# sevagh/xumx-sliCQ

Measured on AMD Instinct MI355X. Metric: real-time factor (audio-s demixed / wall-s), 44.1 kHz stereo, offline model, higher is better.
Workload: dtype f32; 1 GPU; BASELINE configs[1]: offline model (Bark-262 sliCQT), one 240 s stereo track (10,584,000 samples, 5 chunks) per GPU, Wiener off (mix-phase), seeded synthetic weights; parallelism=one track per rank, 1 rank(s), no data-path collective

## Files before the change

### xumx_slicq_amd/csrc/dft_tables.h

```cpp
#pragma once
namespace xsq {
template <int R> struct DftTw;
template <> struct DftTw<43> {
    static constexpr float c[43] = {1.000000000e+00f, 9.893433681e-01f, 9.576005999e-01f, 9.054482375e-01f, 8.339978179e-01f, 7.447721827e-01f, 6.396730216e-01f, 5.209403405e-01f, 3.911047205e-01f, 2.529333824e-01f, 1.093712084e-01f, -3.652202306e-02f, -1.816368510e-01f, -3.228804048e-01f, -4.572423233e-01f, -5.818589156e-01f, -6.940741952e-01f, -7.914964884e-01f, -8.720494081e-01f, -9.340161087e-01f, -9.760758776e-01f, -9.973322837e-01f, -9.973322837e-01f, -9.760758776e-01f, -9.340161087e-01f, -8.720494081e-01f, -7.914964884e-01f, -6.940741952e-01f, -5.818589156e-01f, -4.572423233e-01f, -3.228804048e-01f, -1.816368510e-01f, -3.652202306e-02f, 1.093712084e-01f, 2.529333824e-01f, 3.911047205e-01f, 5.209403405e-01f, 6.396730216e-01f, 7.447721827e-01f, 8.339978179e-01f, 9.054482375e-01f, 9.576005999e-01f, 9.893433681e-01f};
    static constexpr float s[43] = {0.000000000e+00f, 1.456011677e-01f, 2.880990994e-01f, 4.244566989e-01f, 5.517677408e-01f, 6.673188112e-01f, 7.686471398e-01f, 8.535930890e-01f, 9.203461836e-01f, 9.674836971e-01f, 9.940009752e-01f, 9.993328484e-01f, 9.833656768e-01f, 9.464397732e-01f, 8.893421489e-01f, 8.132897407e-01f, 7.199034738e-01f, 6.111737141e-01f, 4.894178478e-01f, 3.572308898e-01f, 2.174301756e-01f, 7.299531466e-02f, -7.299531466e-02f, -2.174301756e-01f, -3.572308898e-01f, -4.894178478e-01f, -6.111737141e-01f, -7.199034738e-01f, -8.132897407e-01f, -8.893421489e-01f, -9.464397732e-01f, -9.833656768e-01f, -9.993328484e-01f, -9.940009752e-01f, -9.674836971e-01f, -9.203461836e-01f, -8.535930890e-01f, -7.686471398e-01f, -6.673188112e-01f, -5.517677408e-01f, -4.244566989e-01f, -2.880990994e-01f, -1.456011677e-01f};
};
template <> struct DftTw<14> {
    static constexpr float c[14] = {1.000000000e+00f, 9.009688679e-01f, 6.234898019e-01f, 2.225209340e-01f, -2.225209340e-01f, -6.234898019e-01f, -9.009688679e-01f, -1.000000000e+00f, -9.009688679e-01f, -6.234898019e-01f, -2.225209340e-01f, 2.225209340e-01f, 6.234898019e-01f, 9.009688679e-01f};
    static constexpr float s[14] = {0.000000000e+00f, 4.338837391e-01f, 7.818314825e-01f, 9.749279122e-01f, 9.749279122e-01f, 7.818314825e-01f, 4.338837391e-01f, 1.224646799e-16f, -4.338837391e-01f, -7.818314825e-01f, -9.749279122e-01f, -9.749279122e-01f, -7.818314825e-01f, -4.338837391e-01f};
};
template <> struct DftTw<15> {
    static constexpr float c[15] = {1.000000000e+00f, 9.135454576e-01f, 6.691306064e-01f, 3.090169944e-01f, -1.045284633e-01f, -5.000000000e-01f, -8.090169944e-01f, -9.781476007e-01f, -9.781476007e-01f, -8.090169944e-01f, -5.000000000e-01f, -1.045284633e-01f, 3.090169944e-01f, 6.691306064e-01f, 9.135454576e-01f};
    static constexpr float s[15] = {0.000000000e+00f, 4.067366431e-01f, 7.431448255e-01f, 9.510565163e-01f, 9.945218954e-01f, 8.660254038e-01f, 5.877852523e-01f, 2.079116908e-01f, -2.079116908e-01f, -5.877852523e-01f, -8.660254038e-01f, -9.945218954e-01f, -9.510565163e-01f, -7.431448255e-01f, -4.067366431e-01f};
};
template <> struct DftTw<4> {
    static constexpr float c[4] = {1.000000000e+00f, 6.123233996e-17f, -1.000000000e+00f, -1.836970199e-16f};
    static constexpr float s[4] = {0.000000000e+00f, 1.000000000e+00f, 1.224646799e-16f, -1.000000000e+00f};
};
template <> struct DftTw<5> {
    static constexpr float c[5] = {1.000000000e+00f, 3.090169944e-01f, -8.090169944e-01f, -8.090169944e-01f, 3.090169944e-01f};
    static constexpr float s[5] = {0.000000000e+00f, 9.510565163e-01f, 5.877852523e-01f, -5.877852523e-01f, -9.510565163e-01f};
};
template <> struct DftTw<6> {
    static constexpr float c[6] = {1.000000000e+00f, 5.000000000e-01f, -5.000000000e-01f, -1.000000000e+00f, -5.000000000e-01f, 5.000000000e-01f};
    static constexpr float s[6] = {0.000000000e+00f, 8.660254038e-01f, 8.660254038e-01f, 1.224646799e-16f, -8.660254038e-01f, -8.660254038e-01f};
};
template <> struct DftTw<7> {
    static constexpr float c[7] = {1.000000000e+00f, 6.234898019e-01f, -2.225209340e-01f, -9.009688679e-01f, -9.009688679e-01f, -2.225209340e-01f, 6.234898019e-01f};
    static constexpr float s[7] = {0.000000000e+00f, 7.818314825e-01f, 9.749279122e-01f, 4.338837391e-01f, -4.338837391e-01f, -9.749279122e-01f, -7.818314825e-01f};
};
template <> struct DftTw<8> {
    static constexpr float c[8] = {1.000000000e+00f, 7.071067812e-01f, 6.123233996e-17f, -7.071067812e-01f, -1.000000000e+00f, -7.071067812e-01f, -1.836970199e-16f, 7.071067812e-01f};
    static constexpr float s[8] = {0.000000000e+00f, 7.071067812e-01f, 1.000000000e+00f, 7.071067812e-01f, 1.224646799e-16f, -7.071067812e-01f, -1.000000000e+00f, -7.071067812e-01f};
};
template <> struct DftTw<9> {
    static constexpr float c[9] = {1.000000000e+00f, 7.660444431e-01f, 1.736481777e-01f, -5.000000000e-01f, -9.396926208e-01f, -9.396926208e-01f, -5.000000000e-01f, 1.736481777e-01f, 7.660444431e-01f};
    static constexpr float s[9] = {0.000000000e+00f, 6.427876097e-01f, 9.848077530e-01f, 8.660254038e-01f, 3.420201433e-01f, -3.420201433e-01f, -8.660254038e-01f, -9.848077530e-01f, -6.427876097e-01f};
};
template <> struct DftTw<10> {
    static constexpr float c[10] = {1.000000000e+00f, 8.090169944e-01f, 3.090169944e-01f, -3.090169944e-01f, -8.090169944e-01f, -1.000000000e+00f, -8.090169944e-01f, -3.090169944e-01f, 3.090169944e-01f, 8.090169944e-01f};
    static constexpr float s[10] = {0.000000000e+00f, 5.877852523e-01f, 9.510565163e-01f, 9.510565163e-01f, 5.877852523e-01f, 1.224646799e-16f, -5.877852523e-01f, -9.510565163e-01f, -9.510565163e-01f, -5.877852523e-01f};
};
template <> struct DftTw<11> {
    static constexpr float c[11] = {1.000000000e+00f, 8.412535328e-01f, 4.154150130e-01f, -1.423148383e-01f, -6.548607339e-01f, -9.594929736e-01f, -9.594929736e-01f, -6.548607339e-01f, -1.423148383e-01f, 4.154150130e-01f, 8.412535328e-01f};
    static constexpr float s[11] = {0.000000000e+00f, 5.406408175e-01f, 9.096319954e-01f, 9.898214419e-01f, 7.557495744e-01f, 2.817325568e-01f, -2.817325568e-01f, -7.557495744e-01f, -9.898214419e-01f, -9.096319954e-01f, -5.406408175e-01f};
};
template <> struct DftTw<12> {
    static constexpr float c[12] = {1.000000000e+00f, 8.660254038e-01f, 5.000000000e-01f, 6.123233996e-17f, -5.000000000e-01f, -8.660254038e-01f, -1.000000000e+00f, -8.660254038e-01f, -5.000000000e-01f, -1.836970199e-16f, 5.000000000e-01f, 8.660254038e-01f};
    static constexpr float s[12] = {0.000000000e+00f, 5.000000000e-01f, 8.660254038e-01f, 1.000000000e+00f, 8.660254038e-01f, 5.000000000e-01f, 1.224646799e-16f, -5.000000000e-01f, -8.660254038e-01f, -1.000000000e+00f, -8.660254038e-01f, -5.000000000e-01f};
};
template <> struct DftTw<13> {
    static constexpr float c[13] = {1.000000000e+00f, 8.854560257e-01f, 5.680647467e-01f, 1.205366803e-01f, -3.546048870e-01f, -7.485107482e-01f, -9.709418174e-01f, -9.709418174e-01f, -7.485107482e-01f, -3.546048870e-01f, 1.205366803e-01f, 5.680647467e-01f, 8.854560257e-01f};
    static constexpr float s[13] = {0.000000000e+00f, 4.647231720e-01f, 8.229838659e-01f, 9.927088741e-01f, 9.350162427e-01f, 6.631226582e-01f, 2.393156643e-01f, -2.393156643e-01f, -6.631226582e-01f, -9.350162427e-01f, -9.927088741e-01f, -8.229838659e-01f, -4.647231720e-01f};
};
}
```

### xumx_slicq_amd/csrc/plan.h

```cpp
#pragma once
#include <map>
#include <mutex>
#include <tuple>
#include <vector>

#include <rocfft/rocfft.h>

#include "common.h"

namespace xsq {

struct FftPlan {
    rocfft_plan plan = nullptr;
    rocfft_execution_info info = nullptr;
    size_t work_bytes = 0;
};

struct TileTable {
    TileDev* d_tiles = nullptr;
    int ntiles = 0;
};

struct BlockHost {
    int first_band, F, T;
    int64_t cum;
};

}

struct xsq_plan {
    int L = 0, tr = 0, h = 0, nbins = 0, nbands = 0, nblocks = 0;
    int64_t sumFT = 0;
    std::vector<xsq::BandDev> bands;
    std::vector<xsq::BlockHost> blocks;
    int band_radix4 = 1;
    void* d_bands4 = nullptr;
    float* d_pool4f = nullptr;
    float* d_pool4i = nullptr;
    int nbands4 = 0;
    std::vector<unsigned char> bands4_host;
    int64_t d4_max_block = 0;
    std::vector<int> bands4_m, bands4_small;
    int fft_backend = 0;
    float2* d_T = nullptr;
    unsigned short* d_tgt16 = nullptr;
    int* d_tgt = nullptr;
    int phase_begin[5] = {0, 0, 0, 0, 0};
    int packed_fft = 0;
    int short_inline = 0;
    void *d_s_item1 = nullptr, *d_s_tw1 = nullptr;
    int *d_s_item2 = nullptr, *d_s_tgt = nullptr;
    float* d_s_wd = nullptr;
    int short_n1 = 0, short_n2 = 0, short_nent = 0, short_sc0 = 0;
    int short_begin[5] = {0, 0, 0, 0, 0};
    int phase_long[4] = {0, 0, 0, 0};
    float* d_tw = nullptr;
    float* d_Wf = nullptr;
    float* d_Wi = nullptr;
    xsq::BandDev* d_bands = nullptr;
    int* d_cov_ptr = nullptr;
    int* d_cov_band = nullptr;
    std::mutex mu;
    std::map<std::pair<int, int>, xsq::FftPlan> fft;
    std::map<std::tuple<int, int, int>, xsq::TileTable> tiles;
};
```

### xumx_slicq_amd/csrc/slicqt.hip

```cpp
#include <algorithm>
#include <cmath>
#include <cstdarg>
#include <cstdio>
#include <cstdlib>
#include <cstring>

#include "../../include/xumx_slicq_hip.h"
#include "gemm_tile.h"
#include "plan.h"
#include "prof.h"
#include "slice_fft.h"
#include "band_dft4.h"
#include "band_dft4s.h"

namespace xsq {

static thread_local char g_err[1024] = "";
void set_error(const char* fmt, ...) {
    va_list ap;
    va_start(ap, fmt);
    vsnprintf(g_err, sizeof(g_err), fmt, ap);
    va_end(ap);
}

__global__ __launch_bounds__(256) void k_slice_window(const float* __restrict__ x,
                                                       const float* __restrict__ tw,
                                                       float* __restrict__ seg, int S, int64_t n, int L,
                                                       int h, const int64_t* __restrict__ xrows = nullptr,
                                                       const float* const* __restrict__ xslot = nullptr) {
    const int p = blockIdx.x * 256 + threadIdx.x;
    if (p >= L) return;
    const int row = blockIdx.y;
    const int bc = row / S, s = row - bc * S;
    const int64_t i = (int64_t)(2 * s - 2) * h + p;
    float v = 0.f;
    if (i >= 0 && i < n) v = tw[p] * (xslot ? *xslot : x)[(xrows ? xrows[bc] : (int64_t)bc * n) + i];
    seg[(int64_t)row * L + p] = v;
}

__global__ __launch_bounds__(256) void k_spectrum_gather(const float* __restrict__ Z,
                                                          const BandDev* __restrict__ bands,
                                                          const int* __restrict__ cov_ptr,
                                                          const int* __restrict__ cov_band,
                                                          float2* __restrict__ fr, int BC, int S, int nbins) {
    const int k = blockIdx.x * 256 + threadIdx.x;
    if (k >= nbins) return;
    const int row = blockIdx.y;
    const int bc = row / S, s = row - bc * S;
    const int64_t BCS = (int64_t)BC * S;
    float2 acc = make_float2(0.f, 0.f);
    for (int e = cov_ptr[k]; e < cov_ptr[k + 1]; ++e) {
        const BandDev b = bands[cov_band[e]];
        const int64_t off = 2 * (BCS * b.cum + (((int64_t)bc * b.F + b.f) * S + s) * b.Lg + (k - b.bin0));
        const float2 z = *reinterpret_cast<const float2*>(Z + off);
        acc.x += z.x;
        acc.y += z.y;
    }
    if (k == 0 || k == nbins - 1) acc.y = 0.f;
    fr[(int64_t)row * nbins + k] = acc;
}

__global__ __launch_bounds__(256) void k_overlap_add(const float* __restrict__ seg, float* __restrict__ y,
                                                      const int64_t* __restrict__ row_off,
                                                      int S, int64_t length, int L, int h) {
    const int64_t i = (int64_t)blockIdx.x * 256 + threadIdx.x;
    if (i >= length) return;
    const int bc = blockIdx.y;
    const int s0 = (int)(i / (2 * h));
    const int p1 = (int)(i - (int64_t)2 * h * s0);
    const float* base = seg + (int64_t)bc * S * L;
    float v = base[(int64_t)s0 * L + p1 + 2 * h];
    if (s0 + 1 < S) v += base[(int64_t)(s0 + 1) * L + p1];
    y[(row_off ? row_off[bc] : (int64_t)bc * length) + i] = v;
}

struct BandGroup {
    int M, N, K, ldb;
    const float* B;
    int Lg, bin0, f, F;
    int64_t base;
    int64_t cum;
    int j;
};

struct BandFwdOp {
    typedef BandGroup Group;
    struct RowA {
        const float* p;
    };
    const float* U;
    float* coef;
    const BandDev* bands;
    const float* W;
    int BC, S, nbins, L;
    float* xin;
    const float* mean;
    const float* scale;
    int split;

    __device__ Group group(int j) const {
        const BandDev b = bands[j];
        Group g;
        g.M = BC * S; g.N = 2 * b.Lg; g.K = 2 * b.Lg; g.ldb = b.ldw; g.B = W + b.w_off;
        g.Lg = b.Lg; g.bin0 = b.bin0; g.f = b.f; g.F = b.F;
        g.base = 2 * ((int64_t)BC * S * b.cum + (int64_t)b.f * S * b.Lg);
        g.cum = b.cum;
        g.j = j;
        return g;
    }
    __device__ RowA row_a(const Group& g, int m) const {
        RowA r;
        r.p = m < g.M ? U + (int64_t)m * 2 * nbins : nullptr;
        return r;
    }
    __device__ float4 load_a4(const Group& g, const RowA& r, int k) const {
        const bool ok = r.p != nullptr && k < g.K;
        int i0 = g.bin0 + (k >> 1), i1 = i0 + 1;
        i0 = i0 < 0 ? -i0 : (i0 > L / 2 ? L - i0 : i0);
        i1 = i1 < 0 ? -i1 : (i1 > L / 2 ? L - i1 : i1);
        const float2 a = *reinterpret_cast<const float2*>(ok ? r.p + 2 * i0 : zero16());
        const float2 b = *reinterpret_cast<const float2*>(ok ? r.p + 2 * i1 : zero16());
        return make_float4(a.x, a.y, b.x, b.y);
    }
    __device__ void epilogue(const Group& g, int row0, int n, const f32x16& a0, const f32x16& a1, bool wide) const {
        const bool c0 = n < g.N, c1 = wide && n + 32 < g.N;
        int bc = row0 / S, s = row0 - bc * S;
        int prev = 0;
        const float mu = xin ? mean[g.j] : 0.f, sc = xin ? scale[g.j] : 1.f;
#pragma unroll
        for (int r = 0; r < 16; ++r) {
            s += acc_row(r) - prev; prev = acc_row(r);
            while (s >= S) { s -= S; ++bc; }
            if (row0 + acc_row(r) >= g.M) break;
            float* d = coef + g.base + ((int64_t)bc * g.F * S + s) * (2 * g.Lg) + n;
            if (c0) d[0] = a0[r];
            if (c1) d[32] = a1[r];
            if (xin) {
                const float o0 = __shfl_xor(a0[r], 1), o1 = __shfl_xor(a1[r], 1);
                if (!(n & 1)) {
                    float* x = xin + ((d - coef) >> 1);
                    if (c0) { float v = whiten_mag(a0[r], o0, mu, sc); if (split) v = bf3_word(v); x[0] = v; }
                    if (c1) { float v = whiten_mag(a1[r], o1, mu, sc); if (split) v = bf3_word(v); x[16] = v; }
                }
            }
        }
    }
};

struct BandInvOp {
    typedef BandGroup Group;
    struct RowA {
        const float* p;
        const float* mk;
    };
    const float* coef;
    float* Z;
    const BandDev* bands;
    const float* W;
    int BC, S;
    int row_len;
    const float* mask;
    int BCx;

    __device__ Group group(int j) const {
        const BandDev b = bands[j];
        Group g;
        g.M = BC * S; g.N = 2 * b.Lg; g.K = 2 * b.Lg; g.ldb = b.ldw; g.B = W + b.w_off;
        g.Lg = b.Lg; g.bin0 = b.ent; g.f = b.f; g.F = b.F;
        g.base = 2 * ((int64_t)BC * S * b.cum + (int64_t)b.f * S * b.Lg);
        g.cum = b.cum;
        return g;
    }
    __device__ int64_t row_off(const Group& g, int m) const {
        const int bc = m / S, s = m - bc * S;
        return g.base + ((int64_t)bc * g.F * S + s) * (2 * g.Lg);
    }
    __device__ RowA row_a(const Group& g, int m) const {
        RowA r;
        r.p = nullptr; r.mk = nullptr;
        if (m >= g.M) return r;
        if (!mask) { r.p = coef + row_off(g, m); return r; }
        const int bc = m / S, s = m - bc * S;
        r.mk = mask + row_off(g, m) / 2;
        r.p = coef + 2 * ((int64_t)BCx * S * g.cum + (int64_t)g.f * S * g.Lg) + ((int64_t)(bc % BCx) * g.F * S + s) * (2 * g.Lg);
        return r;
    }
    __device__ float4 load_a4(const Group& g, const RowA& r, int k) const {
        const bool ok = r.p != nullptr && k < g.K;
        return *reinterpret_cast<const float4*>(ok ? r.p + k : zero16());
    }
    typedef float2 Aux;
    __device__ Aux load_aux(const Group& g, const RowA& r, int k) const {
        const bool ok = r.mk != nullptr && k < g.K;
        return *reinterpret_cast<const float2*>(ok ? r.mk + (k >> 1) : zero16());
    }
    __device__ float4 finish(float4 v, const Aux& mk) const {
        if (mask) { v.x *= mk.x; v.y *= mk.x; v.z *= mk.y; v.w *= mk.y; }
        return v;
    }
    __device__ void epilogue(const Group& g, int row0, int n, const f32x16& a0, const f32x16& a1, bool wide) const {
        const bool c0 = n < g.N, c1 = wide && n + 32 < g.N;
#pragma unroll
        for (int r = 0; r < 16; ++r) {
            const int m = row0 + acc_row(r);
            if (m >= g.M) break;
            float* d = (row_len ? Z + 2 * ((int64_t)m * row_len + g.bin0) : Z + row_off(g, m)) + n;
            if (c0) d[0] = a0[r];
            if (c1) d[32] = a1[r];
        }
    }
};

constexpr int REMIX_MAX_BLOCKS = 256;
struct RemixArgs {
    const float* src;
    float* dst;
    int nch, R, S, cplx;
    float g[4][4];
    int use[4];
    int cum[REMIX_MAX_BLOCKS + 1];
};

__global__ __launch_bounds__(256) void k_remix_combine(RemixArgs a) {
#pragma clang fp contract(off)
    const int j = blockIdx.y, ch = blockIdx.z;
    const int64_t per = (int64_t)a.S * (a.cum[j + 1] - a.cum[j]) * a.cplx;
    const int64_t e = ((int64_t)blockIdx.x * 256 + threadIdx.x) * 4;
    if (e >= per) return;
    const int64_t base = (int64_t)a.S * a.cum[j] * a.cplx;
    const float* s = a.src + base * (4 * a.nch) + (int64_t)ch * per + e;
    float4 m[4];
#pragma unroll
    for (int t = 0; t < 4; ++t)
        m[t] = a.use[t] ? *reinterpret_cast<const float4*>(s + (int64_t)t * a.nch * per) : make_float4(0.f, 0.f, 0.f, 0.f);
    float* d = a.dst + base * ((int64_t)a.R * a.nch) + (int64_t)ch * per + e;
#pragma unroll
    for (int r = 0; r < 4; ++r) {
        if (r >= a.R) break;
        float4 acc = make_float4(0.f, 0.f, 0.f, 0.f);
#pragma unroll
        for (int t = 0; t < 4; ++t) {
            if (!a.use[t]) continue;
            const float g = a.g[r][t];
            acc.x = acc.x + g * m[t].x; acc.y = acc.y + g * m[t].y; acc.z = acc.z + g * m[t].z; acc.w = acc.w + g * m[t].w;
        }
        *reinterpret_cast<float4*>(d + (int64_t)r * a.nch * per) = acc;
    }
}

static int upload_tiles(const std::vector<TileDev>& t, TileTable* tt) {
    tt->ntiles = (int)t.size();
    tt->d_tiles = nullptr;
    if (t.empty()) return XSQ_OK;
    XSQ_HIP(hipMalloc(&tt->d_tiles, t.size() * sizeof(TileDev)));
    XSQ_HIP(hipMemcpy(tt->d_tiles, t.data(), t.size() * sizeof(TileDev), hipMemcpyHostToDevice));
    return XSQ_OK;
}

static int get_band_tiles(xsq_plan* P, int rows, TileTable* out) {
    std::lock_guard<std::mutex> lk(P->mu);
    const bool r4 = P->band_radix4 && P->nbands4 > 0;
    auto key = std::make_tuple(r4 ? 2 : 0, rows, 0);
    auto it = P->tiles.find(key);
    if (it != P->tiles.end()) { *out = it->second; return XSQ_OK; }
    std::vector<TileDev> t;
    if (r4) {
        for (int i = (int)P->bands4_small.size() - 1; i >= 0; --i)
            push_group_tiles(t, P->bands4_small[i], rows, 2 * P->bands[P->bands4_small[i]].Lg);
    } else {
        for (int j = P->nbands - 1; j >= 0; --j) push_group_tiles(t, j, rows, 2 * P->bands[j].Lg);
    }
    TileTable tt;
    int rc = upload_tiles(t, &tt);
    if (rc) return rc;
    P->tiles[key] = tt;
    *out = tt;
    return XSQ_OK;
}

static int get_dft4_full_tiles(xsq_plan* P, int rows, TileTable* out, int share = 0, int cls = 0, bool sym = false) {
    std::lock_guard<std::mutex> lk(P->mu);
    auto key = std::make_tuple(3 + 16 * cls + (sym ? 256 : 0), rows, share);
    auto it = P->tiles.find(key);
    if (it != P->tiles.end()) { *out = it->second; return XSQ_OK; }
    std::vector<Tile4Dev> t;
    const Band4Dev* b4 = reinterpret_cast<const Band4Dev*>(P->bands4_host.data());
    const int span = share > 0 ? share : rows, copies = share > 0 ? rows / share : 1;
    for (int i = P->nbands4 - 1; i >= 0; --i) {
        int ncb = (2 * P->bands4_m[i] + 15) / 16;
        if ((cls == 1 && ncb <= 5) || (cls == 2 && ncb > 5)) continue;
        if (sym) ncb = (P->bands4_m[i] / 2 + 1 + 15) / 16;
        for (int m0 = 0; m0 < span; m0 += D4H_ROWS)
            for (int k = 0; k < copies; ++k) t.push_back(Tile4Dev{m0 + k * span, ncb, b4[i]});
    }
    TileTable tt;
    tt.ntiles = (int)t.size();
    if (!t.empty()) {
        XSQ_HIP(hipMalloc(&tt.d_tiles, t.size() * sizeof(Tile4Dev)));
        XSQ_HIP(hipMemcpy(tt.d_tiles, t.data(), t.size() * sizeof(Tile4Dev), hipMemcpyHostToDevice));
    }
    P->tiles[key] = tt;
    *out = tt;
    return XSQ_OK;
}

static int d4_ranges_ok(const xsq_plan* P, int64_t rows, const char* who) {
    if (!(P->band_radix4 && P->nbands4)) return XSQ_OK;
    XSQ_REQUIRE(8 * rows * P->d4_max_block < (1ll << 30) && (int64_t)8 * D4H_ROWS * std::max<int64_t>(P->nbins, P->sumFT) < (1ll << 30),
                "%s: %lld rows x %lld coefficients of a band block exceed 2^30 bytes; split the call (fewer stacked chunks)",
                who, (long long)rows, (long long)P->d4_max_block);
    return XSQ_OK;
}

template <bool FWD>
static int launch_dft4(xsq_plan* P, const Band4Args& a4, int rows, int share, hipStream_t stream) {
    static const bool split = getenv("XSQ_D4_SPLIT") && atoi(getenv("XSQ_D4_SPLIT")) == 1;
    static const bool sym = !(getenv("XSQ_D4_SYM") && atoi(getenv("XSQ_D4_SYM")) == 0);
    const bool masked = !FWD && a4.mask != nullptr;
    TileTable t;
    int rc;
    if (sym) {
        if ((rc = get_dft4_full_tiles(P, rows, &t, share, 0, true))) return rc;
        if (!t.ntiles) return XSQ_OK;
        if constexpr (!FWD) {
            if (masked) { hipLaunchKernelGGL((band_dft4s_kernel<false, true>), dim3(t.ntiles), dim3(256), 0, stream, a4, (const Tile4Dev*)t.d_tiles, t.ntiles); return XSQ_OK; }
        }
        hipLaunchKernelGGL((band_dft4s_kernel<FWD, false>), dim3(t.ntiles), dim3(256), 0, stream, a4, (const Tile4Dev*)t.d_tiles, t.ntiles);
        return XSQ_OK;
    }
    auto launch = [&](auto ncbmax) {
        constexpr int N = decltype(ncbmax)::value;
        if (!t.ntiles) return;
        if constexpr (!FWD) {
            if (masked) { hipLaunchKernelGGL((band_dft4_full_kernel<false, N, true>), dim3(t.ntiles), dim3(D4H_NT), 0, stream, a4, (const Tile4Dev*)t.d_tiles, t.ntiles); return; }
        }
        hipLaunchKernelGGL((band_dft4_full_kernel<FWD, N, false>), dim3(t.ntiles), dim3(D4H_NT), 0, stream, a4, (const Tile4Dev*)t.d_tiles, t.ntiles);
    };
    if (!split) {
        if ((rc = get_dft4_full_tiles(P, rows, &t, share, 0))) return rc;
        launch(std::integral_constant<int, 10>{});
        return XSQ_OK;
    }
    if ((rc = get_dft4_full_tiles(P, rows, &t, share, 1))) return rc;
    launch(std::integral_constant<int, 10>{});
    if ((rc = get_dft4_full_tiles(P, rows, &t, share, 2))) return rc;
    launch(std::integral_constant<int, 5>{});
    return XSQ_OK;
}

static int get_fft(xsq_plan* P, int inverse, int batch, FftPlan* out) {
    std::lock_guard<std::mutex> lk(P->mu);
    auto key = std::make_pair(inverse, batch);
    auto it = P->fft.find(key);
    if (it != P->fft.end()) {
        *out = it->second;
        return XSQ_OK;
    }
    static std::once_flag once;
    std::call_once(once, [] { rocfft_setup(); });
    FftPlan f;
    size_t len = (size_t)P->L;
    rocfft_status st = rocfft_plan_create(&f.plan, rocfft_placement_notinplace,
                                          inverse ? rocfft_transform_type_real_inverse
                                                  : rocfft_transform_type_real_forward,
                                          rocfft_precision_single, 1, &len, (size_t)batch, nullptr);
    if (st != rocfft_status_success) {
        set_error("rocfft_plan_create(L=%d, batch=%d, inverse=%d) failed: %d", P->L, batch, inverse, (int)st);
        return XSQ_ERR_FFT;
    }
    rocfft_plan_get_work_buffer_size(f.plan, &f.work_bytes);
    if (rocfft_execution_info_create(&f.info) != rocfft_status_success) {
        set_error("rocfft_execution_info_create failed");
        return XSQ_ERR_FFT;
    }
    P->fft[key] = f;
    *out = f;
    return XSQ_OK;
}

static int run_fft(const FftPlan& f, void* in, void* out, void* work, hipStream_t stream) {
    if (rocfft_execution_info_set_stream(f.info, stream) != rocfft_status_success) {
        set_error("rocfft_execution_info_set_stream failed");
        return XSQ_ERR_FFT;
    }
    if (f.work_bytes) {
        if (rocfft_execution_info_set_work_buffer(f.info, work, f.work_bytes) != rocfft_status_success) {
            set_error("rocfft_execution_info_set_work_buffer failed");
            return XSQ_ERR_FFT;
        }
    }
    void* ib[1] = {in};
    void* ob[1] = {out};
    rocfft_status st = rocfft_execute(f.plan, ib, ob, f.info);
    if (st != rocfft_status_success) {
        set_error("rocfft_execute failed: %d", (int)st);
        return XSQ_ERR_FFT;
    }
    return XSQ_OK;
}

static inline size_t al(size_t x) { return (x + 255) / 256 * 256; }

#ifndef XSQ_D4_MIN_LG_DEFAULT
#define XSQ_D4_MIN_LG_DEFAULT 24
#endif
#ifndef XSQ_FFT_NT_FWD
#define XSQ_FFT_NT_FWD 512
#endif
#ifndef XSQ_FFT_NT_INV
#define XSQ_FFT_NT_INV 512
#endif

static int fft_threads(int inverse) {
    static int u[2] = {-1, -1};
    if (u[0] < 0) {
        int f = XSQ_FFT_NT_FWD, i = XSQ_FFT_NT_INV;
        if (const char* e = getenv("XSQ_FFT_THREADS")) { if (sscanf(e, "%d,%d", &f, &i) < 2) i = f; }
        u[0] = f == 512 ? 512 : 256; u[1] = i == 512 ? 512 : 256;
    }
    return u[inverse ? 1 : 0];
}

static inline bool lds_fft(const xsq_plan* P) { return P->fft_backend == 0 && P->L == FFT_L && P->d_tgt != nullptr; }
static inline FftTables fft_tables(const xsq_plan* P) {
    return FftTables{P->d_T, P->d_T + FFT_R1 * FFT_M1, P->d_T + FFT_R1 * FFT_M1 + FFT_R2 * FFT_R3};
}

}

using namespace xsq;

extern "C" {

int xsq_abi_version(void) { return XSQ_ABI_VERSION; }

#ifndef XSQ_BUILD_ARCH
#define XSQ_BUILD_ARCH "unknown"
#endif
#ifndef XSQ_BUILD_FLAGS
#define XSQ_BUILD_FLAGS ""
#endif
const char* xsq_build_info(void) { return "arch=" XSQ_BUILD_ARCH "; flags=" XSQ_BUILD_FLAGS "; date=" __DATE__ " " __TIME__; }
const char* xsq_last_error(void) { return g_err; }

static int plan_build(xsq_plan* P, int L, int tr, int nbands, const int32_t* Lg, const int32_t* c,
                      const float* g, const double* gd, const float* tw);

int xsq_plan_create(xsq_plan** out, int L, int tr, int nbands, const int32_t* Lg, const int32_t* c,
                    const float* g, const double* gd, const float* tw) {
    XSQ_REQUIRE(out && Lg && c && g && gd && tw, "xsq_plan_create: null argument");
    XSQ_REQUIRE(L > 0 && L % 4 == 0 && tr % 2 == 0 && nbands >= 2, "xsq_plan_create: bad L/tr/nbands");
    xsq_plan* P = new xsq_plan();
    const int rc = plan_build(P, L, tr, nbands, Lg, c, g, gd, tw);
    if (rc != XSQ_OK) {
        xsq_plan_destroy(P);
        return rc;
    }
    *out = P;
    return XSQ_OK;
}

static int plan_build(xsq_plan* P, int L, int tr, int nbands, const int32_t* Lg, const int32_t* c,
                      const float* g, const double* gd, const float* tw) {
    P->L = L; P->tr = tr; P->h = L / 4; P->nbins = L / 2 + 1; P->nbands = nbands;
    int64_t cum = 0;
    for (int j = 0; j < nbands;) {
        int k = j;
        while (k + 1 < nbands && Lg[k + 1] == Lg[j]) ++k;
        P->blocks.push_back(BlockHost{j, k - j + 1, Lg[j], cum});
        cum += (int64_t)(k - j + 1) * Lg[j];
        j = k + 1;
    }
    P->nblocks = (int)P->blocks.size();
    P->sumFT = cum;
    int64_t woff = 0, goff = 0;
    std::vector<int64_t> g_off(nbands);
    for (const BlockHost& b : P->blocks) {
        for (int f = 0; f < b.F; ++f) {
            const int j = b.first_band + f;
            if (Lg[j] % 4 != 0 || c[j] % 2 != 0 || Lg[j] > L / 2) {
                set_error("xsq_plan_create: band %d has Lg=%d c=%d (need Lg%%4==0, c even, Lg<=L/2)", j, Lg[j], c[j]);
                return XSQ_ERR_ARG;
            }
            BandDev d;
            d.Lg = Lg[j]; d.bin0 = c[j] - Lg[j] / 2; d.f = f; d.F = b.F; d.cum = b.cum;
            d.ldw = (int)round_up(2 * Lg[j], 16); d.w_off = woff; d.ent = 0;
            woff += round_up(2 * Lg[j], 64) * d.ldw;
            P->bands.push_back(d);
            g_off[j] = goff;
            goff += Lg[j];
        }
    }
    std::vector<float> Wf((size_t)woff, 0.f), Wi((size_t)woff, 0.f);
    const double PI2 = 6.283185307179586476925286766559;
    for (int j = 0; j < nbands; ++j) {
        const BandDev& d = P->bands[j];
        const int n = d.Lg, ld = d.ldw;
        const double sign = ((c[j] / 2) % 2 == 0) ? 1.0 : -1.0;
        std::vector<double> cs(n), sn(n);
        for (int r = 0; r < n; ++r) { cs[r] = std::cos(PI2 * r / n); sn[r] = std::sin(PI2 * r / n); }
        float* wf = Wf.data() + d.w_off;
        float* wi = Wi.data() + d.w_off;
        for (int p = 0; p < n; ++p) {
            const int q = (p + n / 2) % n;
            const int bin = d.bin0 + p;
            const double conj = (bin < 0 || bin > L / 2) ? -1.0 : 1.0;
            const double ga = (double)g[g_off[j] + q] * sign / n;
            const double gs = gd[g_off[j] + q] * n * sign / L;
            for (int t = 0; t < n; ++t) {
                const int r = (int)(((int64_t)q * t) % n);
                const double wr = ga * cs[r], wim = ga * sn[r];
                wf[(size_t)(2 * t) * ld + 2 * p] = (float)wr;
                wf[(size_t)(2 * t + 1) * ld + 2 * p] = (float)wim;
                wf[(size_t)(2 * t) * ld + 2 * p + 1] = (float)(-conj * wim);
                wf[(size_t)(2 * t + 1) * ld + 2 * p + 1] = (float)(conj * wr);
                const double vr = gs * cs[r], vi = -gs * sn[r];
                wi[(size_t)(2 * p) * ld + 2 * t] = (float)vr;
                wi[(size_t)(2 * p + 1) * ld + 2 * t] = (float)vi;
                wi[(size_t)(2 * p) * ld + 2 * t + 1] = (float)(-vi);
                wi[(size_t)(2 * p + 1) * ld + 2 * t + 1] = (float)vr;
            }
        }
    }
    std::vector<int> cov_ptr(P->nbins + 1, 0), cov_band;
    {
        std::vector<std::vector<int>> cov(P->nbins);
        for (int j = 0; j < nbands; ++j)
            for (int p = 0; p < P->bands[j].Lg; ++p) {
                const int k = P->bands[j].bin0 + p;
                if (k >= 0 && k <= L / 2) cov[k].push_back(j);
            }
        for (int k = 0; k < P->nbins; ++k) {
            cov_ptr[k + 1] = cov_ptr[k] + (int)cov[k].size();
            cov_band.insert(cov_band.end(), cov[k].begin(), cov[k].end());
        }
    }
#define UP(dst, vec, T)                                                                           \
    do {                                                                                          \
        XSQ_HIP(hipMalloc(&(dst), (vec).size() * sizeof(T)));                                     \
        XSQ_HIP(hipMemcpy((dst), (vec).data(), (vec).size() * sizeof(T), hipMemcpyHostToDevice)); \
    } while (0)
    UP(P->d_Wf, Wf, float);
    UP(P->d_Wi, Wi, float);
    UP(P->d_bands, P->bands, BandDev);
    UP(P->d_cov_ptr, cov_ptr, int);
    UP(P->d_cov_band, cov_band, int);
#undef UP
    if (L == FFT_L) {
        auto W = [&](int64_t j) {
            j %= L;
            return make_float2((float)std::cos(PI2 * j / L), (float)(-std::sin(PI2 * j / L)));
        };
        std::vector<float2> T;
        for (int k1 = 0; k1 < FFT_R1; ++k1)
            for (int m = 0; m < FFT_M1; ++m) T.push_back(W(2 * (int64_t)k1 * m));
        for (int k2 = 0; k2 < FFT_R2; ++k2)
            for (int n3 = 0; n3 < FFT_R3; ++n3) T.push_back(W(2 * (int64_t)FFT_R1 * n3 * k2));
        for (int k = 0; k <= FFT_N; ++k) T.push_back(W(k));
        XSQ_HIP(hipMalloc(&P->d_T, T.size() * sizeof(float2)));
        XSQ_HIP(hipMemcpy(P->d_T, T.data(), T.size() * sizeof(float2), hipMemcpyHostToDevice));
        std::vector<int> tgt;
        bool ok = true;
        for (int ph = 0; ph < 4; ++ph) {
            P->phase_begin[ph] = (int)tgt.size();
            int last_end = -(1 << 30);
            for (int j = ph; j < nbands; j += 4) {
                BandDev& b = P->bands[j];
                b.ent = (int)tgt.size();
                const int lo = b.bin0 < 0 ? 0 : b.bin0;
                if (lo < last_end) ok = false;
                last_end = b.bin0 + b.Lg > L / 2 + 1 ? L / 2 + 1 : b.bin0 + b.Lg;
                for (int q = 0; q < b.Lg; ++q) {
                    const int k = b.bin0 + q;
                    tgt.push_back(k >= 0 && k <= L / 2 ? k : -1);
                }
            }
        }
        P->phase_begin[4] = (int)tgt.size();
        if (ok) {
            XSQ_HIP(hipMalloc(&P->d_tgt, tgt.size() * sizeof(int)));
            XSQ_HIP(hipMemcpy(P->d_tgt, tgt.data(), tgt.size() * sizeof(int), hipMemcpyHostToDevice));
            std::vector<unsigned short> t16(tgt.size() + 2, 0xFFFFu);
            for (size_t i = 0; i < tgt.size(); ++i) t16[i] = tgt[i] >= 0 ? (unsigned short)tgt[i] : 0xFFFFu;
            XSQ_HIP(hipMalloc(&P->d_tgt16, t16.size() * sizeof(unsigned short)));
            XSQ_HIP(hipMemcpy(P->d_tgt16, t16.data(), t16.size() * sizeof(unsigned short), hipMemcpyHostToDevice));
            XSQ_HIP(hipMemcpy(P->d_bands, P->bands.data(), P->bands.size() * sizeof(BandDev), hipMemcpyHostToDevice));
        }
    }
    {
        std::vector<Band4Dev> b4;
        std::vector<float> pf, pi;
        int d4_min_lg = XSQ_D4_MIN_LG_DEFAULT;
        if (const char* e = getenv("XSQ_D4_MIN_LG")) d4_min_lg = atoi(e) >= 16 ? atoi(e) : d4_min_lg;
        std::map<int, int64_t> doff, twoff, coff;
        auto alloc2 = [&](size_t n) { size_t o = pf.size(); pf.resize(o + n, 0.f); pi.resize(o + n, 0.f); return (int64_t)o; };
        for (int j = 0; j < nbands; ++j) {
            const BandDev& b = P->bands[j];
            if (b.Lg < d4_min_lg || b.Lg > 4 * D4_MPAD) { P->bands4_small.push_back(j); continue; }
            const int n = b.Lg, m = n / 4;
            Band4Dev d;
            memset(&d, 0, sizeof(d));
            d.Lg = n; d.m = m; d.bin0 = b.bin0; d.f = b.f; d.F = b.F; d.ent = b.ent; d.cum = b.cum; d.jband = j;
            d.ldd = (int)round_up(2 * m, 16);
            if (!doff.count(m)) {
                const int64_t o = alloc2((size_t)round_up(2 * m, 64) * d.ldd);
                doff[m] = o;
                for (int k = 0; k < m; ++k)
                    for (int t1 = 0; t1 < m; ++t1) {
                        const int r = (int)(((int64_t)k * t1) % m);
                        const double cr = std::cos(PI2 * r / m), si = std::sin(PI2 * r / m);
                        for (int dir = 0; dir < 2; ++dir) {
                            std::vector<float>& pool = dir ? pi : pf;
                            const double dre = cr, dim = dir ? -si : si;
                            pool[o + (size_t)(2 * k) * d.ldd + 2 * t1] = (float)dre;
                            pool[o + (size_t)(2 * k) * d.ldd + 2 * t1 + 1] = (float)(-dim);
                            pool[o + (size_t)(2 * k + 1) * d.ldd + 2 * t1] = (float)dim;
                            pool[o + (size_t)(2 * k + 1) * d.ldd + 2 * t1 + 1] = (float)dre;
                        }
                    }
            }
            d.d_off = doff[m];
            d.K2 = m / 2 + 1; d.ldc = (int)round_up(d.K2, 8);
            if (!coff.count(m)) {
                const size_t csz = (size_t)round_up(d.K2, 16) * d.ldc;
                const int64_t o = alloc2(2 * csz);
                coff[m] = o;
                for (int k = 0; k < d.K2; ++k)
                    for (int nn = 0; nn < d.K2; ++nn) {
                        const int r = (int)(((int64_t)k * nn) % m);
                        const double cr = std::cos(PI2 * r / m), si = (nn == 0 || 2 * nn == m) ? 0.0 : std::sin(PI2 * r / m);
                        pf[o + (size_t)k * d.ldc + nn] = (float)cr;
                        pi[o + (size_t)k * d.ldc + nn] = (float)cr;
                        pf[o + csz + (size_t)k * d.ldc + nn] = (float)(-si);
                        pi[o + csz + (size_t)k * d.ldc + nn] = (float)si;
                    }
            }
            d.c_off = coff[m];
            if (!twoff.count(n)) {
                const int mpad = (m + 7) & ~7;
                const int64_t o = alloc2((size_t)3 * mpad * 2);
                twoff[n] = o;
                for (int r = 1; r <= 3; ++r)
                    for (int t1 = 0; t1 < m; ++t1) {
                        const int e = (r * t1) % n;
                        const double cr = std::cos(PI2 * e / n), si = std::sin(PI2 * e / n);
                        pf[o + 2 * ((size_t)(r - 1) * mpad + t1)] = (float)cr;
                        pf[o + 2 * ((size_t)(r - 1) * mpad + t1) + 1] = (float)si;
                        pi[o + 2 * ((size_t)(r - 1) * mpad + t1)] = (float)cr;
                        pi[o + 2 * ((size_t)(r - 1) * mpad + t1) + 1] = (float)(-si);
                    }
            }
            d.tw_off = twoff[n];
            d.win_off = alloc2((size_t)round_up(n, 4));
            const double sign = ((c[j] / 2) % 2 == 0) ? 1.0 : -1.0;
            for (int q = 0; q < n; ++q) {
                pf[d.win_off + q] = (float)((double)g[g_off[j] + q] * sign / n);
                pi[d.win_off + q] = (float)(gd[g_off[j] + q] * n * sign / L);
            }
            b4.push_back(d);
            P->bands4_m.push_back(m);
            P->d4_max_block = std::max<int64_t>(P->d4_max_block, (int64_t)b.F * b.Lg);
        }
        P->nbands4 = (int)b4.size();
        P->bands4_host.assign(reinterpret_cast<const unsigned char*>(b4.data()),
                              reinterpret_cast<const unsigned char*>(b4.data()) + b4.size() * sizeof(Band4Dev));
        if (P->nbands4) {
            XSQ_HIP(hipMalloc(&P->d_bands4, b4.size() * sizeof(Band4Dev)));
            XSQ_HIP(hipMemcpy(P->d_bands4, b4.data(), b4.size() * sizeof(Band4Dev), hipMemcpyHostToDevice));
            XSQ_HIP(hipMalloc(&P->d_pool4f, pf.size() * sizeof(float)));
            XSQ_HIP(hipMemcpy(P->d_pool4f, pf.data(), pf.size() * sizeof(float), hipMemcpyHostToDevice));
            XSQ_HIP(hipMalloc(&P->d_pool4i, pi.size() * sizeof(float)));
            XSQ_HIP(hipMemcpy(P->d_pool4i, pi.data(), pi.size() * sizeof(float), hipMemcpyHostToDevice));
        }
    }
    XSQ_HIP(hipMalloc(&P->d_tw, (size_t)L * sizeof(float)));
    XSQ_HIP(hipMemcpy(P->d_tw, tw, (size_t)L * sizeof(float), hipMemcpyHostToDevice));
    if (P->d_tgt != nullptr && P->nbands4 > 0 && !P->bands4_small.empty()) {
        bool ok = true;
        int nent = 0, maxbin = 0;
        for (int j : P->bands4_small) {
            const BandDev& b = P->bands[j];
            if (b.Lg % 4 != 0 || b.Lg < 16 || b.Lg > 60) ok = false;
            nent += b.Lg;
            maxbin = std::max(maxbin, b.bin0 + b.Lg);
        }
        const int sc0 = 4096;
        if (maxbin >= sc0 || sc0 + nent > FFT_N + 1) ok = false;
        if (ok) {
            std::vector<ShortItem1> item1;
            std::vector<float2> tw1;
            std::vector<std::pair<int, int>> item2;
            std::vector<int> stgt((size_t)nent, -1);
            std::vector<float> swd((size_t)nent, 0.f);
            int sc = 0;
            for (int ph = 0; ph < 4; ++ph) {
                P->short_begin[ph] = sc;
                for (int j : P->bands4_small) {
                    if (j % 4 != ph) continue;
                    const BandDev& b = P->bands[j];
                    const int n = b.Lg, m = n / 4;
                    const double sign = ((c[j] / 2) % 2 == 0) ? 1.0 : -1.0;
                    for (int t1 = 0; t1 < m; ++t1) {
                        item1.push_back(ShortItem1{(int)b.cum, b.F, b.f, n, t1, sc});
                        for (int r = 1; r <= 3; ++r) {
                            const int e = (r * t1) % n;
                            tw1.push_back(make_float2((float)std::cos(PI2 * e / n), (float)(-std::sin(PI2 * e / n))));
                        }
                    }
                    for (int r = 0; r < 4; ++r) {
                        item2.push_back({m, ((sc + r * m) << 4) | m});
                        for (int k = 0; k < m; ++k) {
                            const int q = 4 * k + r;
                            const int bin = b.bin0 + (q + n / 2) % n;
                            stgt[sc + r * m + k] = (bin >= 0 && bin <= L / 2) ? bin : -1;
                            swd[sc + r * m + k] = (float)(gd[g_off[j] + q] * n * sign / L);
                        }
                    }
                    sc += n;
                }
            }
            P->short_begin[4] = sc;
            std::stable_sort(item2.begin(), item2.end(), [](const std::pair<int, int>& a, const std::pair<int, int>& b) { return a.first < b.first; });
            std::vector<int> codes;
            for (auto& it : item2) codes.push_back(it.second);
            for (int ph = 0; ph < 4; ++ph) {
                int lo = P->phase_begin[ph + 1];
                for (int j = ph; j < nbands; j += 4) {
                    bool is_short = false;
                    for (int js : P->bands4_small) is_short = is_short || js == j;
                    if (!is_short) { lo = P->bands[j].ent; break; }
                }
                P->phase_long[ph] = lo;
                for (int j = ph; j < nbands; j += 4) {
                    bool is_short = false;
                    for (int js : P->bands4_small) is_short = is_short || js == j;
                    if (is_short && P->bands[j].ent >= lo) ok = false;
                }
            }
            if (ok && item1.size() <= 1280 && codes.size() <= 768 && sc <= nent) {
                bool fits = true;
                for (int ph = 0; ph < 4; ++ph) fits = fits && (P->short_begin[ph + 1] - P->short_begin[ph] <= 1280);
                if (fits) {
#define UPV(dst, vec, T)                                                                          \
    do {                                                                                          \
        XSQ_HIP(hipMalloc((void**)&(dst), (vec).size() * sizeof(T)));                             \
        XSQ_HIP(hipMemcpy((dst), (vec).data(), (vec).size() * sizeof(T), hipMemcpyHostToDevice)); \
    } while (0)
                    UPV(P->d_s_item1, item1, ShortItem1);
                    UPV(P->d_s_tw1, tw1, float2);
                    UPV(P->d_s_item2, codes, int);
                    UPV(P->d_s_tgt, stgt, int);
                    UPV(P->d_s_wd, swd, float);
#undef UPV
                    P->short_n1 = (int)item1.size(); P->short_n2 = (int)codes.size();
                    P->short_nent = nent; P->short_sc0 = sc0;
                }
            }
        }
    }
    return XSQ_OK;
}

int xsq_plan_destroy(xsq_plan* P) {
    if (!P) return XSQ_OK;
    for (auto& kv : P->fft) {
        if (kv.second.info) rocfft_execution_info_destroy(kv.second.info);
        if (kv.second.plan) rocfft_plan_destroy(kv.second.plan);
    }
    for (auto& kv : P->tiles) (void)hipFree(kv.second.d_tiles);
    (void)hipFree(P->d_bands4); (void)hipFree(P->d_pool4f); (void)hipFree(P->d_pool4i);
    (void)hipFree(P->d_T); (void)hipFree(P->d_tgt); (void)hipFree(P->d_tgt16); (void)hipFree(P->d_tw); (void)hipFree(P->d_Wf); (void)hipFree(P->d_Wi); (void)hipFree(P->d_bands);
    (void)hipFree(P->d_cov_ptr); (void)hipFree(P->d_cov_band);
    (void)hipFree(P->d_s_item1); (void)hipFree(P->d_s_tw1); (void)hipFree(P->d_s_item2); (void)hipFree(P->d_s_tgt); (void)hipFree(P->d_s_wd);
    delete P;
    return XSQ_OK;
}

int xsq_plan_num_blocks(const xsq_plan* P) { return P ? P->nblocks : XSQ_ERR_ARG; }

int xsq_plan_set_band_radix4(xsq_plan* P, int on) {
    XSQ_REQUIRE(P, "xsq_plan_set_band_radix4: null plan");
    P->band_radix4 = on ? 1 : 0;
    return XSQ_OK;
}

#if XSQ_D4_STAMP
extern "C" int xsq_debug_d4_stamps(unsigned long long* host, int tiles) {
    XSQ_HIP(hipDeviceSynchronize());
    XSQ_HIP(hipMemcpyFromSymbol(host, HIP_SYMBOL(g_d4_stamps), (size_t)(tiles < D4_STAMP_TILES ? tiles : D4_STAMP_TILES) * 64));
    return XSQ_OK;
}
#endif
#if XSQ_FFT_STAMP
extern "C" int xsq_debug_fft_stamps(unsigned long long* host, int rows) {
    XSQ_HIP(hipDeviceSynchronize());
    XSQ_HIP(hipMemcpyFromSymbol(host, HIP_SYMBOL(g_fft_stamps), (size_t)(rows < FFT_STAMP_ROWS ? rows : FFT_STAMP_ROWS) * 64));
    return XSQ_OK;
}
#endif

int xsq_plan_set_packed_fft(xsq_plan* P, int on) {
    XSQ_REQUIRE(P, "xsq_plan_set_packed_fft: null plan");
#if !XSQ_PACKED_FFT_KERNELS
    XSQ_REQUIRE(!on, "xsq_plan_set_packed_fft: this library is built without the packed-fp32 slice FFT kernels "
                "(diagnostic build: make PACKED_FFT=1)");
#endif
    P->packed_fft = on ? 1 : 0;
    return XSQ_OK;
}

int xsq_plan_set_short_inline(xsq_plan* P, int on) {
    XSQ_REQUIRE(P, "xsq_plan_set_short_inline: null plan");
    P->short_inline = on ? 1 : 0;
    return XSQ_OK;
}

int xsq_plan_set_fft_backend(xsq_plan* P, int backend) {
    XSQ_REQUIRE(P && (backend == 0 || backend == 1), "xsq_plan_set_fft_backend: backend must be 0 (auto) or 1 (rocFFT)");
    P->fft_backend = backend;
    return XSQ_OK;
}

int xsq_plan_block_table(const xsq_plan* P, int64_t* table) {
    XSQ_REQUIRE(P && table, "xsq_plan_block_table: null argument");
    for (int b = 0; b < P->nblocks; ++b) {
        table[4 * b + 0] = P->blocks[b].first_band;
        table[4 * b + 1] = P->blocks[b].F;
        table[4 * b + 2] = P->blocks[b].T;
        table[4 * b + 3] = P->blocks[b].cum;
    }
    return XSQ_OK;
}

int64_t xsq_plan_coefs_per_slice(const xsq_plan* P) { return P ? P->sumFT : XSQ_ERR_ARG; }

int xsq_plan_num_slices(const xsq_plan* P, int64_t n) {
    if (!P || n <= 0) return XSQ_ERR_ARG;
    const int64_t nb = (n + P->h - 1) / P->h;
    return (int)((nb + 1) / 2 + 1);
}

size_t xsq_slicqt_forward_workspace(xsq_plan* P, int BC, int64_t n) {
    if (!P || BC <= 0 || n <= 0) return 0;
    const size_t rows = (size_t)BC * xsq_plan_num_slices(P, n);
    FftPlan f;
    if (!lds_fft(P) && get_fft(P, 0, (int)rows, &f)) return 0;
    return al(rows * P->L * 4) + al(rows * P->nbins * 8) + al(f.work_bytes) + 256;
}

int xsq_slicqt_forward(xsq_plan* P, const float* x, int BC, int64_t n, float* coef, void* ws,
                       size_t ws_bytes, void* stream_) {
    return xsq_slicqt_forward_xin(P, x, BC, n, coef, nullptr, nullptr, nullptr, 0, ws, ws_bytes, stream_);
}

int xsq_slicqt_forward_xin(xsq_plan* P, const float* x, int BC, int64_t n, float* coef, float* xin, const float* mean,
                           const float* scale, int split, void* ws, size_t ws_bytes, void* stream_) {
    return xsq_slicqt_forward_rows(P, x, nullptr, BC, n, n, coef, xin, mean, scale, split, ws, ws_bytes, stream_);
}

int xsq_slicqt_forward_rows(xsq_plan* P, const float* x, const int64_t* x_rows, int BC, int64_t n, int64_t n_pad, float* coef,
                            float* xin, const float* mean, const float* scale, int split, void* ws, size_t ws_bytes,
                            void* stream_) {
    XSQ_REQUIRE(x, "xsq_slicqt_forward: null argument");
    return xsq_slicqt_forward_rows_indirect(P, x, nullptr, x_rows, BC, n, n_pad, coef, xin, mean, scale, split, ws, ws_bytes, stream_);
}

int xsq_slicqt_forward_rows_indirect(xsq_plan* P, const float* x, const float* const* x_slot, const int64_t* x_rows, int BC, int64_t n,
                                     int64_t n_pad, float* coef, float* xin, const float* mean, const float* scale, int split,
                                     void* ws, size_t ws_bytes, void* stream_) {
    XSQ_REQUIRE(P && (x || x_slot) && coef && ws, "xsq_slicqt_forward: null argument");
    XSQ_REQUIRE(!xin || (mean && scale), "xsq_slicqt_forward_xin: xin needs the mean / scale tables");
    XSQ_REQUIRE(BC > 0 && n > 0 && n_pad >= n, "xsq_slicqt_forward: BC=%d n=%lld n_pad=%lld", BC, (long long)n, (long long)n_pad);
    hipStream_t stream = (hipStream_t)stream_;
    const int S = xsq_plan_num_slices(P, n_pad);
    const int rows = BC * S;
    XSQ_REQUIRE(S >= 2, "xsq_slicqt_forward: signal too short");
    XSQ_REQUIRE((int64_t)BC * S <= 65535, "xsq_slicqt_forward: BC*S=%lld rows exceed one launch", (long long)BC * S);
    XSQ_REQUIRE((int64_t)2 * BC * S * (P->sumFT > P->nbins ? P->sumFT : P->nbins) < (1ll << 31),
                "xsq_slicqt_forward: BC*S=%lld rows exceed 2^31 floats of coefficients; split the call", (long long)BC * S);
    if (int rcg = d4_ranges_ok(P, (int64_t)BC * S, "xsq_slicqt_forward")) return rcg;
    FftPlan f;
    int rc = lds_fft(P) ? XSQ_OK : get_fft(P, 0, rows, &f);
    if (rc) return rc;
    char* w = (char*)ws;
    float* seg = (float*)w; w += al((size_t)rows * P->L * 4);
    float* U = (float*)w;   w += al((size_t)rows * P->nbins * 8);
    void* fwork = w;
    if ((size_t)(w - (char*)ws) + f.work_bytes > ws_bytes) {
        set_error("xsq_slicqt_forward: workspace too small (%zu needed, %zu given)",
                  (size_t)(w - (char*)ws) + f.work_bytes, ws_bytes);
        return XSQ_ERR_WORKSPACE;
    }
    if (lds_fft(P)) {
        XSQ_PROF("slice_rfft", stream);
#if XSQ_PACKED_FFT_KERNELS
        if (fft_threads(0) == 512 && P->packed_fft) hipLaunchKernelGGL((k_slice_rfft<512, true>), dim3(rows), dim3(512), 0, stream, x, P->d_tw, fft_tables(P), (float2*)U, S, n, P->h, x_rows, x_slot);
        else
#endif
        if (fft_threads(0) == 512) hipLaunchKernelGGL(k_slice_rfft<512>, dim3(rows), dim3(512), 0, stream, x, P->d_tw, fft_tables(P), (float2*)U, S, n, P->h, x_rows, x_slot);
        else hipLaunchKernelGGL(k_slice_rfft<256>, dim3(rows), dim3(256), 0, stream, x, P->d_tw, fft_tables(P), (float2*)U, S, n, P->h, x_rows, x_slot);
    } else {
        { XSQ_PROF("slice_window", stream);
        hipLaunchKernelGGL(k_slice_window, dim3((P->L + 255) / 256, rows), dim3(256), 0, stream, x, P->d_tw, seg,
                           S, n, P->L, P->h, x_rows, x_slot); }
        { XSQ_PROF("rfft_L", stream); rc = run_fft(f, seg, U, fwork, stream); }
        if (rc) return rc;
    }
    TileTable tt;
    rc = get_band_tiles(P, rows, &tt);
    if (rc) return rc;
    BandFwdOp op{U, coef, P->d_bands, P->d_Wf, BC, S, P->nbins, P->L, xin, mean, scale, split};
    if (P->band_radix4 && P->nbands4) {
        Band4Args a4{(const Band4Dev*)P->d_bands4, P->d_pool4f, U, coef, BC, S, P->nbins, P->L, 0, nullptr, 0, xin, mean, scale, split};
        XSQ_PROF("band_analysis_dft4", stream);
        if ((rc = launch_dft4<true>(P, a4, rows, 0, stream))) return rc;
    }
    if (tt.ntiles) { XSQ_PROF("band_analysis_gemm", stream);
    hipLaunchKernelGGL((grouped_gemm_kernel<BandFwdOp>), dim3(tt.ntiles), dim3(256), 0, stream, op,
                       tt.d_tiles, tt.ntiles); }
    XSQ_HIP(hipGetLastError());
    return XSQ_OK;
}

size_t xsq_slicqt_inverse_workspace(xsq_plan* P, int BC, int S) {
    if (!P || BC <= 0 || S <= 0) return 0;
    const size_t rows = (size_t)BC * S;
    FftPlan f;
    if (!lds_fft(P) && get_fft(P, 1, (int)rows, &f)) return 0;
    if (lds_fft(P)) return al(rows * P->sumFT * 8) + 256;
    return al(rows * P->sumFT * 8) + al(rows * P->nbins * 8) + al(rows * P->L * 4) + al(f.work_bytes) + 256;
}

int xsq_slicqt_inverse(xsq_plan* P, const float* coef, int BC, int S, int64_t length, float* y, void* ws,
                       size_t ws_bytes, void* stream_) {
    return xsq_slicqt_inverse_rows(P, coef, BC, S, length, y, nullptr, ws, ws_bytes, stream_);
}

static int inverse_impl(xsq_plan* P, const float* coef, const float* mask, int BCx, int BC, int S, int64_t length, float* y,
                        const int64_t* row_offsets, void* ws, size_t ws_bytes, void* stream_);

int xsq_slicqt_inverse_rows(xsq_plan* P, const float* coef, int BC, int S, int64_t length, float* y,
                            const int64_t* row_offsets, void* ws, size_t ws_bytes, void* stream_) {
    return inverse_impl(P, coef, nullptr, 0, BC, S, length, y, row_offsets, ws, ws_bytes, stream_);
}

int xsq_slicqt_inverse_masked(xsq_plan* P, const float* masks, const float* mix, int BC, int BCx, int S, int64_t length,
                              float* y, const int64_t* row_offsets, void* ws, size_t ws_bytes, void* stream_) {
    XSQ_REQUIRE(masks && mix, "xsq_slicqt_inverse_masked: null argument");
    XSQ_REQUIRE(BCx > 0 && BC % BCx == 0, "xsq_slicqt_inverse_masked: %d mix channels do not divide %d mask channels", BCx, BC);
    return inverse_impl(P, mix, masks, BCx, BC, S, length, y, row_offsets, ws, ws_bytes, stream_);
}

static int inverse_impl(xsq_plan* P, const float* coef, const float* mask, int BCx, int BC, int S, int64_t length, float* y,
                        const int64_t* row_offsets, void* ws, size_t ws_bytes, void* stream_) {
    XSQ_REQUIRE(P && coef && y && ws, "xsq_slicqt_inverse: null argument");
    XSQ_REQUIRE(BC > 0 && S >= 2 && length > 0, "xsq_slicqt_inverse: BC=%d S=%d length=%lld", BC, S,
                (long long)length);
    XSQ_REQUIRE(length <= (int64_t)2 * S * P->h, "xsq_slicqt_inverse: length %lld exceeds the %d slices",
                (long long)length, S);
    XSQ_REQUIRE((int64_t)BC * S <= 65535, "xsq_slicqt_inverse: BC*S=%lld rows exceed one launch", (long long)BC * S);
    XSQ_REQUIRE((int64_t)2 * BC * S * P->sumFT < (1ll << 31), "xsq_slicqt_inverse: the coefficient arena of BC*S=%lld rows "
                "exceeds 2^31 floats; split the call (fewer stacked chunks)", (long long)BC * S);
    if (int rcg = d4_ranges_ok(P, (int64_t)BC * S, "xsq_slicqt_inverse")) return rcg;
    hipStream_t stream = (hipStream_t)stream_;
    const int rows = BC * S;
    FftPlan f;
    int rc = lds_fft(P) ? XSQ_OK : get_fft(P, 1, rows, &f);
    if (rc) return rc;
    char* w = (char*)ws;
    float* Z = (float*)w;    w += al((size_t)rows * P->sumFT * 8);
    float2* fr = (float2*)w; if (!lds_fft(P)) w += al((size_t)rows * P->nbins * 8);
    float* seg = (float*)w;  if (!lds_fft(P)) w += al((size_t)rows * P->L * 4);
    void* fwork = w;
    if ((size_t)(w - (char*)ws) + f.work_bytes > ws_bytes) {
        set_error("xsq_slicqt_inverse: workspace too small (%zu needed, %zu given)",
                  (size_t)(w - (char*)ws) + f.work_bytes, ws_bytes);
        return XSQ_ERR_WORKSPACE;
    }
    TileTable tt;
    rc = get_band_tiles(P, rows, &tt);
    if (rc) return rc;
    BandInvOp op{coef, Z, P->d_bands, P->d_Wi, BC, S, lds_fft(P) ? (int)P->sumFT : 0, mask, BCx};
    if (P->band_radix4 && P->nbands4) {
        Band4Args a4{(const Band4Dev*)P->d_bands4, P->d_pool4i, coef, Z, BC, S, P->nbins, P->L,
                     lds_fft(P) ? (int)P->sumFT : 0, mask, BCx, nullptr, nullptr, nullptr, 0};
        XSQ_PROF("band_synthesis_dft4", stream);
        if ((rc = launch_dft4<false>(P, a4, rows, mask ? BCx * S : 0, stream))) return rc;
    }
    const bool inl = lds_fft(P) && P->band_radix4 && P->short_inline && P->short_n1 > 0;
    if (tt.ntiles && !inl) { XSQ_PROF("band_synthesis_gemm", stream);
    hipLaunchKernelGGL((grouped_gemm_kernel<BandInvOp>), dim3(tt.ntiles), dim3(256), 0, stream, op,
                       tt.d_tiles, tt.ntiles); }
    if (lds_fft(P)) {
        XSQ_PROF("slice_irfft_ola", stream);
        GatherSched G;
        G.tgt = P->d_tgt; G.tgt16 = P->d_tgt16; G.row_len = (int)P->sumFT;
        for (int i = 0; i < 5; ++i) G.begin[i] = P->phase_begin[i];
        for (int i = 0; i < 4; ++i) G.lo[i] = inl ? P->phase_long[i] : P->phase_begin[i];
        ShortSched SS;
        memset(&SS, 0, sizeof(SS));
        if (inl) {
            SS.item1 = (const ShortItem1*)P->d_s_item1; SS.tw1 = (const float2*)P->d_s_tw1; SS.item2 = P->d_s_item2;
            SS.stgt = P->d_s_tgt; SS.swd = P->d_s_wd;
            SS.n1 = P->short_n1; SS.n2 = P->short_n2; SS.nent = P->short_nent; SS.sc0 = P->short_sc0;
            for (int i = 0; i < 5; ++i) SS.begin[i] = P->short_begin[i];
        }
        const ShortIn SI{coef, mask, BC, mask ? BCx : BC};
        for (int parity = 0; parity < 2; ++parity) {
            const int nsl = (S + 1 - parity) / 2;
            OlaArgs O{y, row_offsets, S, P->h, parity, length};
            const bool sh = SS.n1 > 0;
            bool fast4 = !sh && fft_threads(1) == 512 && G.tgt16 != nullptr && !getenv("XSQ_FFT_GATHER2");
            for (int ph = 0; ph < 4; ++ph) fast4 = fast4 && (G.begin[ph + 1] - (G.lo[ph] & ~1) <= 2 * 512 * ((4864 / 2 + 1 + 511) / 512));
#if XSQ_PACKED_FFT_KERNELS
            if (fast4 && P->packed_fft) hipLaunchKernelGGL((k_slice_irfft<512, true, false, true>), dim3(BC * nsl), dim3(512), 0, stream, (const float2*)Z, G, fft_tables(P), O, SS, SI);
            else if (!fast4 && !sh && fft_threads(1) == 512 && P->packed_fft) hipLaunchKernelGGL((k_slice_irfft<512, true>), dim3(BC * nsl), dim3(512), 0, stream, (const float2*)Z, G, fft_tables(P), O, SS, SI);
            else
#endif
            if (fast4) hipLaunchKernelGGL((k_slice_irfft<512, false, false, true>), dim3(BC * nsl), dim3(512), 0, stream, (const float2*)Z, G, fft_tables(P), O, SS, SI);
            else if (fft_threads(1) == 512 && sh) hipLaunchKernelGGL((k_slice_irfft<512, false, true>), dim3(BC * nsl), dim3(512), 0, stream, (const float2*)Z, G, fft_tables(P), O, SS, SI);
            else if (fft_threads(1) == 512) hipLaunchKernelGGL(k_slice_irfft<512>, dim3(BC * nsl), dim3(512), 0, stream, (const float2*)Z, G, fft_tables(P), O, SS, SI);
            else if (sh) hipLaunchKernelGGL((k_slice_irfft<256, false, true>), dim3(BC * nsl), dim3(256), 0, stream, (const float2*)Z, G, fft_tables(P), O, SS, SI);
            else hipLaunchKernelGGL(k_slice_irfft<256>, dim3(BC * nsl), dim3(256), 0, stream, (const float2*)Z, G, fft_tables(P), O, SS, SI);
        }
        XSQ_HIP(hipGetLastError());
        return XSQ_OK;
    } else {
        { XSQ_PROF("spectrum_gather", stream);
        hipLaunchKernelGGL(k_spectrum_gather, dim3((P->nbins + 255) / 256, rows), dim3(256), 0, stream, Z,
                           P->d_bands, P->d_cov_ptr, P->d_cov_band, fr, BC, S, P->nbins); }
        { XSQ_PROF("irfft_L", stream); rc = run_fft(f, fr, seg, fwork, stream); }
        if (rc) return rc;
    }
    { XSQ_PROF("overlap_add", stream);
    hipLaunchKernelGGL(k_overlap_add, dim3((unsigned)((length + 255) / 256), BC), dim3(256), 0, stream, seg, y,
                       row_offsets, S, length, P->L, P->h); }
    XSQ_HIP(hipGetLastError());
    return XSQ_OK;
}

static int remix_gains_ok(const float* gains, int R, const char* who) {
    XSQ_REQUIRE(gains, "%s: null gains", who);
    XSQ_REQUIRE(R >= 1 && R <= 4, "%s: R=%d mixes (1..4)", who, R);
    for (int i = 0; i < 4 * R; ++i) XSQ_REQUIRE(std::isfinite(gains[i]), "%s: gain [%d][%d] is not finite", who, i / 4, i % 4);
    return XSQ_OK;
}

size_t xsq_slicqt_remix_workspace(xsq_plan* P, int R, int B, int S, int wiener) {
    if (!P || R < 1 || R > 4 || B <= 0 || S <= 0) return 0;
    const size_t inv = xsq_slicqt_inverse_workspace(P, R * 2 * B, S);
    if (!inv) return 0;
    return al((size_t)R * 2 * B * S * P->sumFT * (wiener ? 8 : 4)) + inv;
}

int xsq_slicqt_inverse_remix(xsq_plan* P, const float* masks, const float* mix, const float* Y, const float* gains, int R, int B,
                             int S, int64_t length, float* y, const int64_t* row_offsets, void* ws, size_t ws_bytes, void* stream_) {
    if (int rc = remix_gains_ok(gains, R, "xsq_slicqt_inverse_remix")) return rc;
    XSQ_REQUIRE(P && y && ws, "xsq_slicqt_inverse_remix: null argument");
    XSQ_REQUIRE(Y ? (!masks && !mix) : (masks && mix), "xsq_slicqt_inverse_remix: pass masks and mix (mix-phase) or Y (Wiener-EM), not both");
    XSQ_REQUIRE(B > 0 && S >= 2 && 2 * B <= 65535, "xsq_slicqt_inverse_remix: B=%d S=%d", B, S);
    XSQ_REQUIRE(P->nblocks <= REMIX_MAX_BLOCKS, "xsq_slicqt_inverse_remix: %d band blocks (at most %d)", P->nblocks, REMIX_MAX_BLOCKS);
    const int wiener = Y ? 1 : 0, BC = R * 2 * B;
    const size_t need = xsq_slicqt_remix_workspace(P, R, B, S, wiener);
    XSQ_REQUIRE(need && need <= ws_bytes, "xsq_slicqt_inverse_remix: workspace too small (%zu needed, %zu given)", need, ws_bytes);
    const size_t comb_bytes = al((size_t)BC * S * P->sumFT * (wiener ? 8 : 4));
    float* comb = (float*)ws;
    RemixArgs a;
    a.src = Y ? Y : masks; a.dst = comb; a.nch = 2 * B; a.R = R; a.S = S; a.cplx = wiener ? 2 : 1;
    for (int t = 0; t < 4; ++t) a.use[t] = 0;
    for (int r = 0; r < 4; ++r)
        for (int t = 0; t < 4; ++t) {
            a.g[r][t] = r < R ? gains[4 * r + t] : 0.f;
            if (r < R && gains[4 * r + t] != 0.f) a.use[t] = 1;
        }
    int64_t per_max = 0;
    for (int j = 0; j < P->nblocks; ++j) {
        a.cum[j] = (int)P->blocks[j].cum;
        per_max = std::max<int64_t>(per_max, (int64_t)S * P->blocks[j].F * P->blocks[j].T * a.cplx);
    }
    a.cum[P->nblocks] = (int)P->sumFT;
    hipStream_t stream = (hipStream_t)stream_;
    { XSQ_PROF("remix_combine", stream);
    hipLaunchKernelGGL(k_remix_combine, dim3((unsigned)((per_max / 4 + 255) / 256), P->nblocks, 2 * B), dim3(256), 0, stream, a); }
    XSQ_HIP(hipGetLastError());
    char* inv_ws = (char*)ws + comb_bytes;
    if (wiener) return inverse_impl(P, comb, nullptr, 0, BC, S, length, y, row_offsets, inv_ws, ws_bytes - comb_bytes, stream_);
    return inverse_impl(P, mix, comb, 2 * B, BC, S, length, y, row_offsets, inv_ws, ws_bytes - comb_bytes, stream_);
}

}
```

Measured before the change: 55340 x real-time.

## Add register/LDS radix-4 FFT kernel for mid-size bands in inverse synthesis

Adds a wave-per-16-rows kernel that computes the inverse band transform for bands of length 16 to 60 as a radix-4 by small-DFT factorisation, using per-wave LDS staging and compile-time twiddles. Those bands are taken out of the dense GEMM and dft4 tile tables on the synthesis path, replacing an O(n^2) matrix product with an FFT. The change adds a new kernel launch, per-m template instantiations with extra register pressure, and new tile tables keyed on the mask-sharing layout.

```diff
diff --git a/xumx_slicq_amd/csrc/band_fft_reg.h b/xumx_slicq_amd/csrc/band_fft_reg.h
--- /dev/null
+++ b/xumx_slicq_amd/csrc/band_fft_reg.h
@@ -0,0 +1,142 @@
+#pragma once
+#include "band_dft4.h"
+#include "slice_fft.h"
+
+#ifndef XSQ_BAND_REGFFT_MAX_LG
+#define XSQ_BAND_REGFFT_MAX_LG 60
+#endif
+#ifndef XSQ_BAND_REGFFT_ABL
+#define XSQ_BAND_REGFFT_ABL 0
+#endif
+
+namespace xsq {
+
+constexpr int RF_WROWS = 16, RF_WAVES = 4, RF_ROWS = RF_WROWS * RF_WAVES;
+constexpr int RF_MAX_LG = 60, RF_LDS_W = RF_WROWS * (RF_MAX_LG + 1);
+static_assert(XSQ_BAND_REGFFT_MAX_LG <= RF_MAX_LG, "dft_small codelets exist for m <= 15");
+
+__device__ __forceinline__ void rf_wave_sync() {
+    __builtin_amdgcn_fence(__ATOMIC_RELEASE, "wavefront");
+    __builtin_amdgcn_wave_barrier();
+    __builtin_amdgcn_fence(__ATOMIC_ACQUIRE, "wavefront");
+}
+
+template <bool MASKED, int M_>
+__device__ __forceinline__ void band_fft_reg_body(const Band4Args& a, const Tile4Dev& t, float2* __restrict__ lw, int lane, int w0, int nrows) {
+#pragma clang fp contract(off)
+    constexpr int Lg = 4 * M_, LD = Lg + 1, HP = Lg / 2;
+    constexpr int NP = (RF_WROWS * HP + 63) / 64;
+    constexpr bool FULL = NP * 64 == RF_WROWS * HP;
+    const Band4Dev& bd = t.bd;
+    const int M = a.BC * a.S;
+    const int64_t BCS = (int64_t)a.BC * a.S;
+    const unsigned blk = (unsigned)(bd.F * Lg) * (unsigned)a.S;
+
+    const int myrow = t.m0 + w0 + (lane & 15);
+    const bool my_ok = (lane & 15) < nrows && myrow < M;
+    const int rowc = my_ok ? myrow : 0;
+    const int bc = rowc / a.S, sl = rowc - bc * a.S;
+    const unsigned o_arena = my_ok ? 8u * (unsigned)(((bc * bd.F + bd.f) * a.S + sl) * Lg) : BUF_OOB;
+    unsigned o_src = o_arena, o_msk = BUF_OOB;
+    if (MASKED) {
+        o_src = my_ok ? 8u * (unsigned)((((bc % a.BCx) * bd.F + bd.f) * a.S + sl) * Lg) : BUF_OOB;
+        o_msk = my_ok ? 4u * (unsigned)(((bc * bd.F + bd.f) * a.S + sl) * Lg) : BUF_OOB;
+    }
+    const bool rowmajor = a.row_len != 0;
+    const unsigned o_dst = rowmajor ? (my_ok ? 8u * (unsigned)((w0 + (lane & 15)) * a.row_len) : BUF_OOB) : o_arena;
+    const float* const win = a.pool + bd.win_off;
+
+    const __amdgpu_buffer_rsrc_t rx = MASKED ? buf_rsrc(a.src + 2 * ((int64_t)a.BCx * a.S * bd.cum), 8u * a.BCx * blk)
+                                             : buf_rsrc(a.src + 2 * (BCS * bd.cum), 8u * a.BC * blk);
+    const __amdgpu_buffer_rsrc_t rm = MASKED ? buf_rsrc(a.mask + BCS * bd.cum, 4u * a.BC * blk) : buf_rsrc(a.src, 0);
+    float4 v[NP];
+    float2 mk[NP];
+    float2 wd[NP];
+#pragma unroll
+    for (int u = 0; u < NP; ++u) {
+        const int i = lane + 64 * u, row = i / HP, pr = i - row * HP;
+        const bool ok = FULL || i < RF_WROWS * HP;
+        const unsigned ro = (unsigned)__shfl((int)o_src, row & 15);
+        v[u] = buf_ld4(rx, ok ? ro + 16u * (unsigned)pr : BUF_OOB, 0);
+        wd[u] = *reinterpret_cast<const float2*>(win + 2 * pr);
+        if (MASKED) {
+            const unsigned mo = (unsigned)__shfl((int)o_msk, row & 15);
+            mk[u] = buf_ld2(rm, ok ? mo + 8u * (unsigned)pr : BUF_OOB, 0);
+        }
+    }
+#pragma unroll
+    for (int u = 0; u < NP; ++u) {
+        const int i = lane + 64 * u, row = i / HP, pr = i - row * HP;
+        if (!FULL && i >= RF_WROWS * HP) continue;
+        float4 x = v[u];
+        if (MASKED) { x.x *= mk[u].x; x.y *= mk[u].x; x.z *= mk[u].y; x.w *= mk[u].y; }
+        lw[row * LD + 2 * pr] = make_float2(x.x, x.y);
+        lw[row * LD + 2 * pr + 1] = make_float2(x.z, x.w);
+    }
+    rf_wave_sync();
+
+    const int lrow = lane >> 2, r = lane & 3;
+    const bool odd = r & 1;
+    const float s2 = odd ? -1.f : 1.f;
+    const float cx = odd ? (r == 3 ? -1.f : 1.f) : (r == 2 ? -1.f : 1.f);
+    const float cy = odd ? (r == 3 ? 1.f : -1.f) : (r == 2 ? -1.f : 1.f);
+    const float f0 = r == 0 ? 1.f : 0.f, f1 = r == 1 ? 1.f : 0.f, f2 = r == 2 ? 1.f : 0.f, f3 = r == 3 ? 1.f : 0.f;
+    float2* const xr = lw + lrow * LD;
+    float2 y[M_];
+    static_for<0, M_>([&](auto t1c) {
+        constexpr int t1 = t1c;
+        const float2 x0 = xr[t1], x1 = xr[M_ + t1], x2 = xr[2 * M_ + t1], x3 = xr[3 * M_ + t1];
+        const float2 uu = make_float2(fmaf(s2, x2.x, x0.x), fmaf(s2, x2.y, x0.y));
+        const float2 vv = make_float2(fmaf(s2, x3.x, x1.x), fmaf(s2, x3.y, x1.y));
+        const float pp = odd ? vv.y : vv.x, qq = odd ? vv.x : vv.y;
+        const float2 yy = make_float2(fmaf(cx, pp, uu.x), fmaf(cy, qq, uu.y));
+        if constexpr (t1 == 0) {
+            y[t1] = yy;
+        } else {
+            constexpr float c1 = DftTw<Lg>::c[t1], c2 = DftTw<Lg>::c[2 * t1 % Lg], c3 = DftTw<Lg>::c[3 * t1 % Lg];
+            constexpr float s1 = -DftTw<Lg>::s[t1], s2_ = -DftTw<Lg>::s[2 * t1 % Lg], s3 = -DftTw<Lg>::s[3 * t1 % Lg];
+            const float wx = fmaf(f1, c1, fmaf(f2, c2, fmaf(f3, c3, f0)));
+            const float wy = fmaf(f1, s1, fmaf(f2, s2_, f3 * s3));
+            y[t1] = make_float2(fmaf(yy.x, wx, -(yy.y * wy)), fmaf(yy.x, wy, yy.y * wx));
+        }
+    });
+    rf_wave_sync();
+    dft_small<M_, -1>(y, [&](int k, float2 X) {
+        const int q = 4 * k + r;
+        xr[q < 2 * M_ ? q + 2 * M_ : q - 2 * M_] = X;
+    });
+    rf_wave_sync();
+
+    const float* const dbase = rowmajor ? a.dst + 2 * ((int64_t)t.m0 * a.row_len + bd.ent) : a.dst + 2 * (BCS * bd.cum);
+    const unsigned dbytes = rowmajor ? 8u * (unsigned)(RF_ROWS * a.row_len) : 8u * a.BC * blk;
+    const __amdgpu_buffer_rsrc_t rd = buf_rsrc(dbase, dbytes);
+#pragma unroll
+    for (int u = 0; u < NP; ++u) {
+        const int i = lane + 64 * u, row = i / HP, pr = i - row * HP;
+        const unsigned ro = (unsigned)__shfl((int)o_dst, row & 15);
+        if (!FULL && i >= RF_WROWS * HP) continue;
+        const float2 c0 = lw[row * LD + 2 * pr], c1 = lw[row * LD + 2 * pr + 1];
+        const float4 o = make_float4(c0.x * wd[u].x, c0.y * wd[u].x, c1.x * wd[u].y, c1.y * wd[u].y);
+        buf_st4(o, rd, ro + 16u * (unsigned)pr, 0);
+    }
+}
+
+template <bool MASKED>
+__global__ __launch_bounds__(64 * RF_WAVES) __attribute__((amdgpu_waves_per_eu(4)))
+void band_fft_reg_kernel(Band4Args a, const Tile4Dev* __restrict__ tiles, int ntiles) {
+    __shared__ __attribute__((aligned(16))) float2 lds[RF_WAVES * RF_LDS_W];
+    const int lane = threadIdx.x & 63, wave = threadIdx.x >> 6;
+    const Tile4Dev t = tiles[xcd_remap(blockIdx.x, ntiles)];
+    const int w0 = RF_WROWS * wave, nrows = t.ncb - w0;
+    if (nrows <= 0) return;
+    float2* const lw = lds + wave * RF_LDS_W;
+    switch (t.bd.m) {
+#define XSQ_RF_CASE(MM) case MM: band_fft_reg_body<MASKED, MM>(a, t, lw, lane, w0, nrows); break;
+        XSQ_RF_CASE(4) XSQ_RF_CASE(5) XSQ_RF_CASE(6) XSQ_RF_CASE(7) XSQ_RF_CASE(8) XSQ_RF_CASE(9)
+        XSQ_RF_CASE(10) XSQ_RF_CASE(11) XSQ_RF_CASE(12) XSQ_RF_CASE(13) XSQ_RF_CASE(14) XSQ_RF_CASE(15)
+#undef XSQ_RF_CASE
+        default: break;
+    }
+}
+
+}
diff --git a/xumx_slicq_amd/csrc/dft_tables.h b/xumx_slicq_amd/csrc/dft_tables.h
--- a/xumx_slicq_amd/csrc/dft_tables.h
+++ b/xumx_slicq_amd/csrc/dft_tables.h
@@ -53,4 +53,52 @@
     static constexpr float c[13] = {1.000000000e+00f, 8.854560257e-01f, 5.680647467e-01f, 1.205366803e-01f, -3.546048870e-01f, -7.485107482e-01f, -9.709418174e-01f, -9.709418174e-01f, -7.485107482e-01f, -3.546048870e-01f, 1.205366803e-01f, 5.680647467e-01f, 8.854560257e-01f};
     static constexpr float s[13] = {0.000000000e+00f, 4.647231720e-01f, 8.229838659e-01f, 9.927088741e-01f, 9.350162427e-01f, 6.631226582e-01f, 2.393156643e-01f, -2.393156643e-01f, -6.631226582e-01f, -9.350162427e-01f, -9.927088741e-01f, -8.229838659e-01f, -4.647231720e-01f};
 };
+template <> struct DftTw<16> {
+    static constexpr float c[16] = {1.000000000e+00f, 9.238795325e-01f, 7.071067812e-01f, 3.826834324e-01f, 6.123233996e-17f, -3.826834324e-01f, -7.071067812e-01f, -9.238795325e-01f, -1.000000000e+00f, -9.238795325e-01f, -7.071067812e-01f, -3.826834324e-01f, -1.836970199e-16f, 3.826834324e-01f, 7.071067812e-01f, 9.238795325e-01f};
+    static constexpr float s[16] = {0.000000000e+00f, 3.826834324e-01f, 7.071067812e-01f, 9.238795325e-01f, 1.000000000e+00f, 9.238795325e-01f, 7.071067812e-01f, 3.826834324e-01f, 1.224646799e-16f, -3.826834324e-01f, -7.071067812e-01f, -9.238795325e-01f, -1.000000000e+00f, -9.238795325e-01f, -7.071067812e-01f, -3.826834324e-01f};
+};
+template <> struct DftTw<20> {
+    static constexpr float c[20] = {1.000000000e+00f, 9.510565163e-01f, 8.090169944e-01f, 5.877852523e-01f, 3.090169944e-01f, 6.123233996e-17f, -3.090169944e-01f, -5.877852523e-01f, -8.090169944e-01f, -9.510565163e-01f, -1.000000000e+00f, -9.510565163e-01f, -8.090169944e-01f, -5.877852523e-01f, -3.090169944e-01f, -1.836970199e-16f, 3.090169944e-01f, 5.877852523e-01f, 8.090169944e-01f, 9.510565163e-01f};
+    static constexpr float s[20] = {0.000000000e+00f, 3.090169944e-01f, 5.877852523e-01f, 8.090169944e-01f, 9.510565163e-01f, 1.000000000e+00f, 9.510565163e-01f, 8.090169944e-01f, 5.877852523e-01f, 3.090169944e-01f, 1.224646799e-16f, -3.090169944e-01f, -5.877852523e-01f, -8.090169944e-01f, -9.510565163e-01f, -1.000000000e+00f, -9.510565163e-01f, -8.090169944e-01f, -5.877852523e-01f, -3.090169944e-01f};
+};
+template <> struct DftTw<24> {
+    static constexpr float c[24] = {1.000000000e+00f, 9.659258263e-01f, 8.660254038e-01f, 7.071067812e-01f, 5.000000000e-01f, 2.588190451e-01f, 6.123233996e-17f, -2.588190451e-01f, -5.000000000e-01f, -7.071067812e-01f, -8.660254038e-01f, -9.659258263e-01f, -1.000000000e+00f, -9.659258263e-01f, -8.660254038e-01f, -7.071067812e-01f, -5.000000000e-01f, -2.588190451e-01f, -1.836970199e-16f, 2.588190451e-01f, 5.000000000e-01f, 7.071067812e-01f, 8.660254038e-01f, 9.659258263e-01f};
+    static constexpr float s[24] = {0.000000000e+00f, 2.588190451e-01f, 5.000000000e-01f, 7.071067812e-01f, 8.660254038e-01f, 9.659258263e-01f, 1.000000000e+00f, 9.659258263e-01f, 8.660254038e-01f, 7.071067812e-01f, 5.000000000e-01f, 2.588190451e-01f, 1.224646799e-16f, -2.588190451e-01f, -5.000000000e-01f, -7.071067812e-01f, -8.660254038e-01f, -9.659258263e-01f, -1.000000000e+00f, -9.659258263e-01f, -8.660254038e-01f, -7.071067812e-01f, -5.000000000e-01f, -2.588190451e-01f};
+};
+template <> struct DftTw<28> {
+    static constexpr float c[28] = {1.000000000e+00f, 9.749279122e-01f, 9.009688679e-01f, 7.818314825e-01f, 6.234898019e-01f, 4.338837391e-01f, 2.225209340e-01f, 6.123233996e-17f, -2.225209340e-01f, -4.338837391e-01f, -6.234898019e-01f, -7.818314825e-01f, -9.009688679e-01f, -9.749279122e-01f, -1.000000000e+00f, -9.749279122e-01f, -9.009688679e-01f, -7.818314825e-01f, -6.234898019e-01f, -4.338837391e-01f, -2.225209340e-01f, -1.836970199e-16f, 2.225209340e-01f, 4.338837391e-01f, 6.234898019e-01f, 7.818314825e-01f, 9.009688679e-01f, 9.749279122e-01f};
+    static constexpr float s[28] = {0.000000000e+00f, 2.225209340e-01f, 4.338837391e-01f, 6.234898019e-01f, 7.818314825e-01f, 9.009688679e-01f, 9.749279122e-01f, 1.000000000e+00f, 9.749279122e-01f, 9.009688679e-01f, 7.818314825e-01f, 6.234898019e-01f, 4.338837391e-01f, 2.225209340e-01f, 1.224646799e-16f, -2.225209340e-01f, -4.338837391e-01f, -6.234898019e-01f, -7.818314825e-01f, -9.009688679e-01f, -9.749279122e-01f, -1.000000000e+00f, -9.749279122e-01f, -9.009688679e-01f, -7.818314825e-01f, -6.234898019e-01f, -4.338837391e-01f, -2.225209340e-01f};
+};
+template <> struct DftTw<32> {
+    static constexpr float c[32] = {1.000000000e+00f, 9.807852804e-01f, 9.238795325e-01f, 8.314696123e-01f, 7.071067812e-01f, 5.555702330e-01f, 3.826834324e-01f, 1.950903220e-01f, 6.123233996e-17f, -1.950903220e-01f, -3.826834324e-01f, -5.555702330e-01f, -7.071067812e-01f, -8.314696123e-01f, -9.238795325e-01f, -9.807852804e-01f, -1.000000000e+00f, -9.807852804e-01f, -9.238795325e-01f, -8.314696123e-01f, -7.071067812e-01f, -5.555702330e-01f, -3.826834324e-01f, -1.950903220e-01f, -1.836970199e-16f, 1.950903220e-01f, 3.826834324e-01f, 5.555702330e-01f, 7.071067812e-01f, 8.314696123e-01f, 9.238795325e-01f, 9.807852804e-01f};
+    static constexpr float s[32] = {0.000000000e+00f, 1.950903220e-01f, 3.826834324e-01f, 5.555702330e-01f, 7.071067812e-01f, 8.314696123e-01f, 9.238795325e-01f, 9.807852804e-01f, 1.000000000e+00f, 9.807852804e-01f, 9.238795325e-01f, 8.314696123e-01f, 7.071067812e-01f, 5.555702330e-01f, 3.826834324e-01f, 1.950903220e-01f, 1.224646799e-16f, -1.950903220e-01f, -3.826834324e-01f, -5.555702330e-01f, -7.071067812e-01f, -8.314696123e-01f, -9.238795325e-01f, -9.807852804e-01f, -1.000000000e+00f, -9.807852804e-01f, -9.238795325e-01f, -8.314696123e-01f, -7.071067812e-01f, -5.555702330e-01f, -3.826834324e-01f, -1.950903220e-01f};
+};
+template <> struct DftTw<36> {
+    static constexpr float c[36] = {1.000000000e+00f, 9.848077530e-01f, 9.396926208e-01f, 8.660254038e-01f, 7.660444431e-01f, 6.427876097e-01f, 5.000000000e-01f, 3.420201433e-01f, 1.736481777e-01f, 6.123233996e-17f, -1.736481777e-01f, -3.420201433e-01f, -5.000000000e-01f, -6.427876097e-01f, -7.660444431e-01f, -8.660254038e-01f, -9.396926208e-01f, -9.848077530e-01f, -1.000000000e+00f, -9.848077530e-01f, -9.396926208e-01f, -8.660254038e-01f, -7.660444431e-01f, -6.427876097e-01f, -5.000000000e-01f, -3.420201433e-01f, -1.736481777e-01f, -1.836970199e-16f, 1.736481777e-01f, 3.420201433e-01f, 5.000000000e-01f, 6.427876097e-01f, 7.660444431e-01f, 8.660254038e-01f, 9.396926208e-01f, 9.848077530e-01f};
+    static constexpr float s[36] = {0.000000000e+00f, 1.736481777e-01f, 3.420201433e-01f, 5.000000000e-01f, 6.427876097e-01f, 7.660444431e-01f, 8.660254038e-01f, 9.396926208e-01f, 9.848077530e-01f, 1.000000000e+00f, 9.848077530e-01f, 9.396926208e-01f, 8.660254038e-01f, 7.660444431e-01f, 6.427876097e-01f, 5.000000000e-01f, 3.420201433e-01f, 1.736481777e-01f, 1.224646799e-16f, -1.736481777e-01f, -3.420201433e-01f, -5.000000000e-01f, -6.427876097e-01f, -7.660444431e-01f, -8.660254038e-01f, -9.396926208e-01f, -9.848077530e-01f, -1.000000000e+00f, -9.848077530e-01f, -9.396926208e-01f, -8.660254038e-01f, -7.660444431e-01f, -6.427876097e-01f, -5.000000000e-01f, -3.420201433e-01f, -1.736481777e-01f};
+};
+template <> struct DftTw<40> {
+    static constexpr float c[40] = {1.000000000e+00f, 9.876883406e-01f, 9.510565163e-01f, 8.910065242e-01f, 8.090169944e-01f, 7.071067812e-01f, 5.877852523e-01f, 4.539904997e-01f, 3.090169944e-01f, 1.564344650e-01f, 6.123233996e-17f, -1.564344650e-01f, -3.090169944e-01f, -4.539904997e-01f, -5.877852523e-01f, -7.071067812e-01f, -8.090169944e-01f, -8.910065242e-01f, -9.510565163e-01f, -9.876883406e-01f, -1.000000000e+00f, -9.876883406e-01f, -9.510565163e-01f, -8.910065242e-01f, -8.090169944e-01f, -7.071067812e-01f, -5.877852523e-01f, -4.539904997e-01f, -3.090169944e-01f, -1.564344650e-01f, -1.836970199e-16f, 1.564344650e-01f, 3.090169944e-01f, 4.539904997e-01f, 5.877852523e-01f, 7.071067812e-01f, 8.090169944e-01f, 8.910065242e-01f, 9.510565163e-01f, 9.876883406e-01f};
+    static constexpr float s[40] = {0.000000000e+00f, 1.564344650e-01f, 3.090169944e-01f, 4.539904997e-01f, 5.877852523e-01f, 7.071067812e-01f, 8.090169944e-01f, 8.910065242e-01f, 9.510565163e-01f, 9.876883406e-01f, 1.000000000e+00f, 9.876883406e-01f, 9.510565163e-01f, 8.910065242e-01f, 8.090169944e-01f, 7.071067812e-01f, 5.877852523e-01f, 4.539904997e-01f, 3.090169944e-01f, 1.564344650e-01f, 1.224646799e-16f, -1.564344650e-01f, -3.090169944e-01f, -4.539904997e-01f, -5.877852523e-01f, -7.071067812e-01f, -8.090169944e-01f, -8.910065242e-01f, -9.510565163e-01f, -9.876883406e-01f, -1.000000000e+00f, -9.876883406e-01f, -9.510565163e-01f, -8.910065242e-01f, -8.090169944e-01f, -7.071067812e-01f, -5.877852523e-01f, -4.539904997e-01f, -3.090169944e-01f, -1.564344650e-01f};
+};
+template <> struct DftTw<44> {
+    static constexpr float c[44] = {1.000000000e+00f, 9.898214419e-01f, 9.594929736e-01f, 9.096319954e-01f, 8.412535328e-01f, 7.557495744e-01f, 6.548607339e-01f, 5.406408175e-01f, 4.154150130e-01f, 2.817325568e-01f, 1.423148383e-01f, 2.832769449e-16f, -1.423148383e-01f, -2.817325568e-01f, -4.154150130e-01f, -5.406408175e-01f, -6.548607339e-01f, -7.557495744e-01f, -8.412535328e-01f, -9.096319954e-01f, -9.594929736e-01f, -9.898214419e-01f, -1.000000000e+00f, -9.898214419e-01f, -9.594929736e-01f, -9.096319954e-01f, -8.412535328e-01f, -7.557495744e-01f, -6.548607339e-01f, -5.406408175e-01f, -4.154150130e-01f, -2.817325568e-01f, -1.423148383e-01f, -1.836970199e-16f, 1.423148383e-01f, 2.817325568e-01f, 4.154150130e-01f, 5.406408175e-01f, 6.548607339e-01f, 7.557495744e-01f, 8.412535328e-01f, 9.096319954e-01f, 9.594929736e-01f, 9.898214419e-01f};
+    static constexpr float s[44] = {0.000000000e+00f, 1.423148383e-01f, 2.817325568e-01f, 4.154150130e-01f, 5.406408175e-01f, 6.548607339e-01f, 7.557495744e-01f, 8.412535328e-01f, 9.096319954e-01f, 9.594929736e-01f, 9.898214419e-01f, 1.000000000e+00f, 9.898214419e-01f, 9.594929736e-01f, 9.096319954e-01f, 8.412535328e-01f, 7.557495744e-01f, 6.548607339e-01f, 5.406408175e-01f, 4.154150130e-01f, 2.817325568e-01f, 1.423148383e-01f, 5.665538898e-16f, -1.423148383e-01f, -2.817325568e-01f, -4.154150130e-01f, -5.406408175e-01f, -6.548607339e-01f, -7.557495744e-01f, -8.412535328e-01f, -9.096319954e-01f, -9.594929736e-01f, -9.898214419e-01f, -1.000000000e+00f, -9.898214419e-01f, -9.594929736e-01f, -9.096319954e-01f, -8.412535328e-01f, -7.557495744e-01f, -6.548607339e-01f, -5.406408175e-01f, -4.154150130e-01f, -2.817325568e-01f, -1.423148383e-01f};
+};
+template <> struct DftTw<48> {
+    static constexpr float c[48] = {1.000000000e+00f, 9.914448614e-01f, 9.659258263e-01f, 9.238795325e-01f, 8.660254038e-01f, 7.933533403e-01f, 7.071067812e-01f, 6.087614290e-01f, 5.000000000e-01f, 3.826834324e-01f, 2.588190451e-01f, 1.305261922e-01f, 6.123233996e-17f, -1.305261922e-01f, -2.588190451e-01f, -3.826834324e-01f, -5.000000000e-01f, -6.087614290e-01f, -7.071067812e-01f, -7.933533403e-01f, -8.660254038e-01f, -9.238795325e-01f, -9.659258263e-01f, -9.914448614e-01f, -1.000000000e+00f, -9.914448614e-01f, -9.659258263e-01f, -9.238795325e-01f, -8.660254038e-01f, -7.933533403e-01f, -7.071067812e-01f, -6.087614290e-01f, -5.000000000e-01f, -3.826834324e-01f, -2.588190451e-01f, -1.305261922e-01f, -1.836970199e-16f, 1.305261922e-01f, 2.588190451e-01f, 3.826834324e-01f, 5.000000000e-01f, 6.087614290e-01f, 7.071067812e-01f, 7.933533403e-01f, 8.660254038e-01f, 9.238795325e-01f, 9.659258263e-01f, 9.914448614e-01f};
+    static constexpr float s[48] = {0.000000000e+00f, 1.305261922e-01f, 2.588190451e-01f, 3.826834324e-01f, 5.000000000e-01f, 6.087614290e-01f, 7.071067812e-01f, 7.933533403e-01f, 8.660254038e-01f, 9.238795325e-01f, 9.659258263e-01f, 9.914448614e-01f, 1.000000000e+00f, 9.914448614e-01f, 9.659258263e-01f, 9.238795325e-01f, 8.660254038e-01f, 7.933533403e-01f, 7.071067812e-01f, 6.087614290e-01f, 5.000000000e-01f, 3.826834324e-01f, 2.588190451e-01f, 1.305261922e-01f, 1.224646799e-16f, -1.305261922e-01f, -2.588190451e-01f, -3.826834324e-01f, -5.000000000e-01f, -6.087614290e-01f, -7.071067812e-01f, -7.933533403e-01f, -8.660254038e-01f, -9.238795325e-01f, -9.659258263e-01f, -9.914448614e-01f, -1.000000000e+00f, -9.914448614e-01f, -9.659258263e-01f, -9.238795325e-01f, -8.660254038e-01f, -7.933533403e-01f, -7.071067812e-01f, -6.087614290e-01f, -5.000000000e-01f, -3.826834324e-01f, -2.588190451e-01f, -1.305261922e-01f};
+};
+template <> struct DftTw<52> {
+    static constexpr float c[52] = {1.000000000e+00f, 9.927088741e-01f, 9.709418174e-01f, 9.350162427e-01f, 8.854560257e-01f, 8.229838659e-01f, 7.485107482e-01f, 6.631226582e-01f, 5.680647467e-01f, 4.647231720e-01f, 3.546048870e-01f, 2.393156643e-01f, 1.205366803e-01f, -1.608122650e-16f, -1.205366803e-01f, -2.393156643e-01f, -3.546048870e-01f, -4.647231720e-01f, -5.680647467e-01f, -6.631226582e-01f, -7.485107482e-01f, -8.229838659e-01f, -8.854560257e-01f, -9.350162427e-01f, -9.709418174e-01f, -9.927088741e-01f, -1.000000000e+00f, -9.927088741e-01f, -9.709418174e-01f, -9.350162427e-01f, -8.854560257e-01f, -8.229838659e-01f, -7.485107482e-01f, -6.631226582e-01f, -5.680647467e-01f, -4.647231720e-01f, -3.546048870e-01f, -2.393156643e-01f, -1.205366803e-01f, -1.836970199e-16f, 1.205366803e-01f, 2.393156643e-01f, 3.546048870e-01f, 4.647231720e-01f, 5.680647467e-01f, 6.631226582e-01f, 7.485107482e-01f, 8.229838659e-01f, 8.854560257e-01f, 9.350162427e-01f, 9.709418174e-01f, 9.927088741e-01f};
+    static constexpr float s[52] = {0.000000000e+00f, 1.205366803e-01f, 2.393156643e-01f, 3.546048870e-01f, 4.647231720e-01f, 5.680647467e-01f, 6.631226582e-01f, 7.485107482e-01f, 8.229838659e-01f, 8.854560257e-01f, 9.350162427e-01f, 9.709418174e-01f, 9.927088741e-01f, 1.000000000e+00f, 9.927088741e-01f, 9.709418174e-01f, 9.350162427e-01f, 8.854560257e-01f, 8.229838659e-01f, 7.485107482e-01f, 6.631226582e-01f, 5.680647467e-01f, 4.647231720e-01f, 3.546048870e-01f, 2.393156643e-01f, 1.205366803e-01f, -3.216245299e-16f, -1.205366803e-01f, -2.393156643e-01f, -3.546048870e-01f, -4.647231720e-01f, -5.680647467e-01f, -6.631226582e-01f, -7.485107482e-01f, -8.229838659e-01f, -8.854560257e-01f, -9.350162427e-01f, -9.709418174e-01f, -9.927088741e-01f, -1.000000000e+00f, -9.927088741e-01f, -9.709418174e-01f, -9.350162427e-01f, -8.854560257e-01f, -8.229838659e-01f, -7.485107482e-01f, -6.631226582e-01f, -5.680647467e-01f, -4.647231720e-01f, -3.546048870e-01f, -2.393156643e-01f, -1.205366803e-01f};
+};
+template <> struct DftTw<56> {
+    static constexpr float c[56] = {1.000000000e+00f, 9.937122099e-01f, 9.749279122e-01f, 9.438833303e-01f, 9.009688679e-01f, 8.467241992e-01f, 7.818314825e-01f, 7.071067812e-01f, 6.234898019e-01f, 5.320320765e-01f, 4.338837391e-01f, 3.302790620e-01f, 2.225209340e-01f, 1.119644761e-01f, 6.123233996e-17f, -1.119644761e-01f, -2.225209340e-01f, -3.302790620e-01f, -4.338837391e-01f, -5.320320765e-01f, -6.234898019e-01f, -7.071067812e-01f, -7.818314825e-01f, -8.467241992e-01f, -9.009688679e-01f, -9.438833303e-01f, -9.749279122e-01f, -9.937122099e-01f, -1.000000000e+00f, -9.937122099e-01f, -9.749279122e-01f, -9.438833303e-01f, -9.009688679e-01f, -8.467241992e-01f, -7.818314825e-01f, -7.071067812e-01f, -6.234898019e-01f, -5.320320765e-01f, -4.338837391e-01f, -3.302790620e-01f, -2.225209340e-01f, -1.119644761e-01f, -1.836970199e-16f, 1.119644761e-01f, 2.225209340e-01f, 3.302790620e-01f, 4.338837391e-01f, 5.320320765e-01f, 6.234898019e-01f, 7.071067812e-01f, 7.818314825e-01f, 8.467241992e-01f, 9.009688679e-01f, 9.438833303e-01f, 9.749279122e-01f, 9.937122099e-01f};
+    static constexpr float s[56] = {0.000000000e+00f, 1.119644761e-01f, 2.225209340e-01f, 3.302790620e-01f, 4.338837391e-01f, 5.320320765e-01f, 6.234898019e-01f, 7.071067812e-01f, 7.818314825e-01f, 8.467241992e-01f, 9.009688679e-01f, 9.438833303e-01f, 9.749279122e-01f, 9.937122099e-01f, 1.000000000e+00f, 9.937122099e-01f, 9.749279122e-01f, 9.438833303e-01f, 9.009688679e-01f, 8.467241992e-01f, 7.818314825e-01f, 7.071067812e-01f, 6.234898019e-01f, 5.320320765e-01f, 4.338837391e-01f, 3.302790620e-01f, 2.225209340e-01f, 1.119644761e-01f, 1.224646799e-16f, -1.119644761e-01f, -2.225209340e-01f, -3.302790620e-01f, -4.338837391e-01f, -5.320320765e-01f, -6.234898019e-01f, -7.071067812e-01f, -7.818314825e-01f, -8.467241992e-01f, -9.009688679e-01f, -9.438833303e-01f, -9.749279122e-01f, -9.937122099e-01f, -1.000000000e+00f, -9.937122099e-01f, -9.749279122e-01f, -9.438833303e-01f, -9.009688679e-01f, -8.467241992e-01f, -7.818314825e-01f, -7.071067812e-01f, -6.234898019e-01f, -5.320320765e-01f, -4.338837391e-01f, -3.302790620e-01f, -2.225209340e-01f, -1.119644761e-01f};
+};
+template <> struct DftTw<60> {
+    static constexpr float c[60] = {1.000000000e+00f, 9.945218954e-01f, 9.781476007e-01f, 9.510565163e-01f, 9.135454576e-01f, 8.660254038e-01f, 8.090169944e-01f, 7.431448255e-01f, 6.691306064e-01f, 5.877852523e-01f, 5.000000000e-01f, 4.067366431e-01f, 3.090169944e-01f, 2.079116908e-01f, 1.045284633e-01f, 2.832769449e-16f, -1.045284633e-01f, -2.079116908e-01f, -3.090169944e-01f, -4.067366431e-01f, -5.000000000e-01f, -5.877852523e-01f, -6.691306064e-01f, -7.431448255e-01f, -8.090169944e-01f, -8.660254038e-01f, -9.135454576e-01f, -9.510565163e-01f, -9.781476007e-01f, -9.945218954e-01f, -1.000000000e+00f, -9.945218954e-01f, -9.781476007e-01f, -9.510565163e-01f, -9.135454576e-01f, -8.660254038e-01f, -8.090169944e-01f, -7.431448255e-01f, -6.691306064e-01f, -5.877852523e-01f, -5.000000000e-01f, -4.067366431e-01f, -3.090169944e-01f, -2.079116908e-01f, -1.045284633e-01f, -1.836970199e-16f, 1.045284633e-01f, 2.079116908e-01f, 3.090169944e-01f, 4.067366431e-01f, 5.000000000e-01f, 5.877852523e-01f, 6.691306064e-01f, 7.431448255e-01f, 8.090169944e-01f, 8.660254038e-01f, 9.135454576e-01f, 9.510565163e-01f, 9.781476007e-01f, 9.945218954e-01f};
+    static constexpr float s[60] = {0.000000000e+00f, 1.045284633e-01f, 2.079116908e-01f, 3.090169944e-01f, 4.067366431e-01f, 5.000000000e-01f, 5.877852523e-01f, 6.691306064e-01f, 7.431448255e-01f, 8.090169944e-01f, 8.660254038e-01f, 9.135454576e-01f, 9.510565163e-01f, 9.781476007e-01f, 9.945218954e-01f, 1.000000000e+00f, 9.945218954e-01f, 9.781476007e-01f, 9.510565163e-01f, 9.135454576e-01f, 8.660254038e-01f, 8.090169944e-01f, 7.431448255e-01f, 6.691306064e-01f, 5.877852523e-01f, 5.000000000e-01f, 4.067366431e-01f, 3.090169944e-01f, 2.079116908e-01f, 1.045284633e-01f, 5.665538898e-16f, -1.045284633e-01f, -2.079116908e-01f, -3.090169944e-01f, -4.067366431e-01f, -5.000000000e-01f, -5.877852523e-01f, -6.691306064e-01f, -7.431448255e-01f, -8.090169944e-01f, -8.660254038e-01f, -9.135454576e-01f, -9.510565163e-01f, -9.781476007e-01f, -9.945218954e-01f, -1.000000000e+00f, -9.945218954e-01f, -9.781476007e-01f, -9.510565163e-01f, -9.135454576e-01f, -8.660254038e-01f, -8.090169944e-01f, -7.431448255e-01f, -6.691306064e-01f, -5.877852523e-01f, -5.000000000e-01f, -4.067366431e-01f, -3.090169944e-01f, -2.079116908e-01f, -1.045284633e-01f};
+};
 }
diff --git a/xumx_slicq_amd/csrc/plan.h b/xumx_slicq_amd/csrc/plan.h
--- a/xumx_slicq_amd/csrc/plan.h
+++ b/xumx_slicq_amd/csrc/plan.h
@@ -41,6 +41,9 @@
     std::vector<unsigned char> bands4_host;
     int64_t d4_max_block = 0;
     std::vector<int> bands4_m, bands4_small;
+    std::vector<unsigned char> bandsr_host;
+    std::vector<char> band_reg;
+    int nbandsr = 0;
     int fft_backend = 0;
     float2* d_T = nullptr;
     unsigned short* d_tgt16 = nullptr;
diff --git a/xumx_slicq_amd/csrc/slicqt.hip b/xumx_slicq_amd/csrc/slicqt.hip
--- a/xumx_slicq_amd/csrc/slicqt.hip
+++ b/xumx_slicq_amd/csrc/slicqt.hip
@@ -12,6 +12,7 @@
 #include "slice_fft.h"
 #include "band_dft4.h"
 #include "band_dft4s.h"
+#include "band_fft_reg.h"
 
 namespace xsq {
 
@@ -257,16 +258,24 @@
     return XSQ_OK;
 }
 
-static int get_band_tiles(xsq_plan* P, int rows, TileTable* out) {
+static inline bool reg_class_on(const xsq_plan* P, bool fwd) {
+    return !fwd && P->band_radix4 && P->nbandsr > 0;
+}
+
+enum { TK_DENSE_ALL = 0, TK_DENSE_SHORT = 2, TK_DFT4 = 3 , TK_REGFFT = 5, TK_SKIP_REG = 8, TK_SYM = 256, TK_SKIP_SMALL = 1024 };
+
+static int get_band_tiles(xsq_plan* P, int rows, TileTable* out, bool fwd) {
     std::lock_guard<std::mutex> lk(P->mu);
-    const bool r4 = P->band_radix4 && P->nbands4 > 0;
-    auto key = std::make_tuple(r4 ? 2 : 0, rows, 0);
+    const bool reg = reg_class_on(P, fwd);
+    const bool r4 = P->band_radix4 && (P->nbands4 > 0 || reg);
+    auto key = std::make_tuple((r4 ? TK_DENSE_SHORT : TK_DENSE_ALL) + (reg ? TK_SKIP_REG : 0), rows, 0);
     auto it = P->tiles.find(key);
     if (it != P->tiles.end()) { *out = it->second; return XSQ_OK; }
     std::vector<TileDev> t;
     if (r4) {
         for (int i = (int)P->bands4_small.size() - 1; i >= 0; --i)
-            push_group_tiles(t, P->bands4_small[i], rows, 2 * P->bands[P->bands4_small[i]].Lg);
+            if (!(reg && P->band_reg[P->bands4_small[i]]))
+                push_group_tiles(t, P->bands4_small[i], rows, 2 * P->bands[P->bands4_small[i]].Lg);
     } else {
         for (int j = P->nbands - 1; j >= 0; --j) push_group_tiles(t, j, rows, 2 * P->bands[j].Lg);
     }
@@ -278,9 +287,9 @@
     return XSQ_OK;
 }
 
-static int get_dft4_full_tiles(xsq_plan* P, int rows, TileTable* out, int share = 0, int cls = 0, bool sym = false) {
+static int get_dft4_full_tiles(xsq_plan* P, int rows, TileTable* out, bool skip_reg, int share = 0, int cls = 0, bool sym = false) {
     std::lock_guard<std::mutex> lk(P->mu);
-    auto key = std::make_tuple(3 + 16 * cls + (sym ? 256 : 0), rows, share);
+    auto key = std::make_tuple(TK_DFT4 + 16 * cls + (sym ? TK_SYM : 0) + (skip_reg ? TK_SKIP_REG : 0), rows, share);
     auto it = P->tiles.find(key);
     if (it != P->tiles.end()) { *out = it->second; return XSQ_OK; }
     std::vector<Tile4Dev> t;
@@ -289,6 +298,7 @@
     for (int i = P->nbands4 - 1; i >= 0; --i) {
         int ncb = (2 * P->bands4_m[i] + 15) / 16;
         if ((cls == 1 && ncb <= 5) || (cls == 2 && ncb > 5)) continue;
+        if (skip_reg && P->band_reg[b4[i].jband]) continue;
         if (sym) ncb = (P->bands4_m[i] / 2 + 1 + 15) / 16;
         for (int m0 = 0; m0 < span; m0 += D4H_ROWS)
             for (int k = 0; k < copies; ++k) t.push_back(Tile4Dev{m0 + k * span, ncb, b4[i]});
@@ -304,9 +314,35 @@
     return XSQ_OK;
 }
 
+static int get_reg_tiles(xsq_plan* P, int rows, TileTable* out, int share, bool skip_small) {
+    std::lock_guard<std::mutex> lk(P->mu);
+    auto key = std::make_tuple(TK_REGFFT + (skip_small ? TK_SKIP_SMALL : 0), rows, share);
+    auto it = P->tiles.find(key);
+    if (it != P->tiles.end()) { *out = it->second; return XSQ_OK; }
+    std::vector<Tile4Dev> t;
+    const Band4Dev* br = reinterpret_cast<const Band4Dev*>(P->bandsr_host.data());
+    const int span = share > 0 ? share : rows, copies = share > 0 ? rows / share : 1;
+    std::vector<char> small(P->nbands, 0);
+    for (int j : P->bands4_small) small[j] = 1;
+    for (int i = P->nbandsr - 1; i >= 0; --i) {
+        if (skip_small && small[br[i].jband]) continue;
+        for (int m0 = 0; m0 < span; m0 += RF_ROWS)
+            for (int k = 0; k < copies; ++k) t.push_back(Tile4Dev{m0 + k * span, std::min(RF_ROWS, span - m0), br[i]});
+    }
+    TileTable tt;
+    tt.ntiles = (int)t.size();
+    if (!t.empty()) {
+        XSQ_HIP(hipMalloc(&tt.d_tiles, t.size() * sizeof(Tile4Dev)));
+        XSQ_HIP(hipMemcpy(tt.d_tiles, t.data(), t.size() * sizeof(Tile4Dev), hipMemcpyHostToDevice));
+    }
+    P->tiles[key] = tt;
+    *out = tt;
+    return XSQ_OK;
+}
+
 static int d4_ranges_ok(const xsq_plan* P, int64_t rows, const char* who) {
-    if (!(P->band_radix4 && P->nbands4)) return XSQ_OK;
-    XSQ_REQUIRE(8 * rows * P->d4_max_block < (1ll << 30) && (int64_t)8 * D4H_ROWS * std::max<int64_t>(P->nbins, P->sumFT) < (1ll << 30),
+    if (!(P->band_radix4 && (P->nbands4 || P->nbandsr))) return XSQ_OK;
+    XSQ_REQUIRE(8 * rows * P->d4_max_block < (1ll << 30) && (int64_t)8 * std::max(D4H_ROWS, RF_ROWS) * std::max<int64_t>(P->nbins, P->sumFT) < (1ll << 30),
                 "%s: %lld rows x %lld coefficients of a band block exceed 2^30 bytes; split the call (fewer stacked chunks)",
                 who, (long long)rows, (long long)P->d4_max_block);
     return XSQ_OK;
@@ -317,10 +353,11 @@
     static const bool split = getenv("XSQ_D4_SPLIT") && atoi(getenv("XSQ_D4_SPLIT")) == 1;
     static const bool sym = !(getenv("XSQ_D4_SYM") && atoi(getenv("XSQ_D4_SYM")) == 0);
     const bool masked = !FWD && a4.mask != nullptr;
+    const bool skip_reg = reg_class_on(P, FWD);
     TileTable t;
     int rc;
     if (sym) {
-        if ((rc = get_dft4_full_tiles(P, rows, &t, share, 0, true))) return rc;
+        if ((rc = get_dft4_full_tiles(P, rows, &t, skip_reg, share, 0, true))) return rc;
         if (!t.ntiles) return XSQ_OK;
         if constexpr (!FWD) {
             if (masked) { hipLaunchKernelGGL((band_dft4s_kernel<false, true>), dim3(t.ntiles), dim3(256), 0, stream, a4, (const Tile4Dev*)t.d_tiles, t.ntiles); return XSQ_OK; }
@@ -337,13 +374,13 @@
         hipLaunchKernelGGL((band_dft4_full_kernel<FWD, N, false>), dim3(t.ntiles), dim3(D4H_NT), 0, stream, a4, (const Tile4Dev*)t.d_tiles, t.ntiles);
     };
     if (!split) {
-        if ((rc = get_dft4_full_tiles(P, rows, &t, share, 0))) return rc;
+        if ((rc = get_dft4_full_tiles(P, rows, &t, skip_reg, share, 0))) return rc;
         launch(std::integral_constant<int, 10>{});
         return XSQ_OK;
     }
-    if ((rc = get_dft4_full_tiles(P, rows, &t, share, 1))) return rc;
+    if ((rc = get_dft4_full_tiles(P, rows, &t, skip_reg, share, 1))) return rc;
     launch(std::integral_constant<int, 10>{});
-    if ((rc = get_dft4_full_tiles(P, rows, &t, share, 2))) return rc;
+    if ((rc = get_dft4_full_tiles(P, rows, &t, skip_reg, share, 2))) return rc;
     launch(std::integral_constant<int, 5>{});
     return XSQ_OK;
 }
@@ -661,12 +698,36 @@
             P->bands4_m.push_back(m);
             P->d4_max_block = std::max<int64_t>(P->d4_max_block, (int64_t)b.F * b.Lg);
         }
+        std::vector<Band4Dev> br;
+        P->band_reg.assign(nbands, 0);
+        for (int j = 0; j < nbands; ++j) {
+            const BandDev& b = P->bands[j];
+            if (b.Lg < 16 || b.Lg > XSQ_BAND_REGFFT_MAX_LG) continue;
+            const int n = b.Lg, m = n / 4;
+            Band4Dev d;
+            memset(&d, 0, sizeof(d));
+            d.Lg = n; d.m = m; d.bin0 = b.bin0; d.f = b.f; d.F = b.F; d.ent = b.ent; d.cum = b.cum; d.jband = j;
+            d.win_off = alloc2((size_t)n);
+            const double sign = ((c[j] / 2) % 2 == 0) ? 1.0 : -1.0;
+            for (int p = 0; p < n; ++p) {
+                const int q = (p + n / 2) % n;
+                pi[d.win_off + p] = (float)(gd[g_off[j] + q] * n * sign / L);
+            }
+            br.push_back(d);
+            P->band_reg[j] = 1;
+            P->d4_max_block = std::max<int64_t>(P->d4_max_block, (int64_t)b.F * b.Lg);
+        }
+        P->nbandsr = (int)br.size();
+        P->bandsr_host.assign(reinterpret_cast<const unsigned char*>(br.data()),
+                              reinterpret_cast<const unsigned char*>(br.data()) + br.size() * sizeof(Band4Dev));
         P->nbands4 = (int)b4.size();
         P->bands4_host.assign(reinterpret_cast<const unsigned char*>(b4.data()),
                               reinterpret_cast<const unsigned char*>(b4.data()) + b4.size() * sizeof(Band4Dev));
         if (P->nbands4) {
             XSQ_HIP(hipMalloc(&P->d_bands4, b4.size() * sizeof(Band4Dev)));
             XSQ_HIP(hipMemcpy(P->d_bands4, b4.data(), b4.size() * sizeof(Band4Dev), hipMemcpyHostToDevice));
+        }
+        if (P->nbands4 || P->nbandsr) {
             XSQ_HIP(hipMalloc(&P->d_pool4f, pf.size() * sizeof(float)));
             XSQ_HIP(hipMemcpy(P->d_pool4f, pf.data(), pf.size() * sizeof(float), hipMemcpyHostToDevice));
             XSQ_HIP(hipMalloc(&P->d_pool4i, pi.size() * sizeof(float)));
@@ -907,7 +968,7 @@
         if (rc) return rc;
     }
     TileTable tt;
-    rc = get_band_tiles(P, rows, &tt);
+    rc = get_band_tiles(P, rows, &tt, true);
     if (rc) return rc;
     BandFwdOp op{U, coef, P->d_bands, P->d_Wf, BC, S, P->nbins, P->L, xin, mean, scale, split};
     if (P->band_radix4 && P->nbands4) {
@@ -978,19 +1039,27 @@
         return XSQ_ERR_WORKSPACE;
     }
     TileTable tt;
-    rc = get_band_tiles(P, rows, &tt);
+    rc = get_band_tiles(P, rows, &tt, false);
     if (rc) return rc;
     BandInvOp op{coef, Z, P->d_bands, P->d_Wi, BC, S, lds_fft(P) ? (int)P->sumFT : 0, mask, BCx};
+    const Band4Args a4{(const Band4Dev*)P->d_bands4, P->d_pool4i, coef, Z, BC, S, P->nbins, P->L,
+                       lds_fft(P) ? (int)P->sumFT : 0, mask, BCx, nullptr, nullptr, nullptr, 0};
+    const bool inl = lds_fft(P) && P->band_radix4 && P->short_inline && P->short_n1 > 0;
+    TileTable tr;
+    if (reg_class_on(P, false) && (rc = get_reg_tiles(P, rows, &tr, mask ? BCx * S : 0, inl))) return rc;
     if (P->band_radix4 && P->nbands4) {
-        Band4Args a4{(const Band4Dev*)P->d_bands4, P->d_pool4i, coef, Z, BC, S, P->nbins, P->L,
-                     lds_fft(P) ? (int)P->sumFT : 0, mask, BCx, nullptr, nullptr, nullptr, 0};
         XSQ_PROF("band_synthesis_dft4", stream);
         if ((rc = launch_dft4<false>(P, a4, rows, mask ? BCx * S : 0, stream))) return rc;
     }
-    const bool inl = lds_fft(P) && P->band_radix4 && P->short_inline && P->short_n1 > 0;
-    if (tt.ntiles && !inl) { XSQ_PROF("band_synthesis_gemm", stream);
-    hipLaunchKernelGGL((grouped_gemm_kernel<BandInvOp>), dim3(tt.ntiles), dim3(256), 0, stream, op,
-                       tt.d_tiles, tt.ntiles); }
+    if ((tt.ntiles && !inl) || tr.ntiles) {
+        XSQ_PROF("band_synthesis_gemm", stream);
+        if (tr.ntiles && !XSQ_BAND_REGFFT_ABL) {
+            if (mask) hipLaunchKernelGGL((band_fft_reg_kernel<true>), dim3(tr.ntiles), dim3(64 * RF_WAVES), 0, stream, a4, (const Tile4Dev*)tr.d_tiles, tr.ntiles);
+            else hipLaunchKernelGGL((band_fft_reg_kernel<false>), dim3(tr.ntiles), dim3(64 * RF_WAVES), 0, stream, a4, (const Tile4Dev*)tr.d_tiles, tr.ntiles);
+        }
+        if (tt.ntiles && !inl)
+            hipLaunchKernelGGL((grouped_gemm_kernel<BandInvOp>), dim3(tt.ntiles), dim3(256), 0, stream, op, tt.d_tiles, tt.ntiles);
+    }
     if (lds_fft(P)) {
         XSQ_PROF("slice_irfft_ola", stream);
         GatherSched G;
```

Result: faster. 56190 x real-time (median of 6 runs) (+1.5%).
